# NVIDIA/audio-flamingo

Hardware: AMD Instinct MI355X
Metric: audio-sec/s + decoder tokens/s, AF3-7B bf16 train (higher is better)
Workload: dtype bf16; 1 GPU; AF3 (AF-Whisper 32L + Qwen2.5-7B 28L, MLP projector) bf16 train step fwd+bwd+AdamW, 30 s clips, S=1024; micro_batch_per_gpu=8, global_batch=8, seq_len=1024, parallelism=dp1, activation_checkpointing=False

## Files before the change

### audio-flamingo_amd/csrc/ceiling.hip

```cpp
#include "common.h"
#include "../../include/afk.h"

namespace {

constexpr int SEG = 16;

template <int MODE>
__global__ __launch_bounds__(512, 1) void mfma_ceiling_kernel(const bf16* __restrict__ src, float* __restrict__ sink, int iters) {
    extern __shared__ __attribute__((aligned(16))) char smem[];
    const int tid = threadIdx.x, lane = tid & 63, wave = tid >> 6;
    bf16x8 a[2][4], b[2][4];
    const bf16x8* s8 = (const bf16x8*)src;
#pragma unroll
    for (int i = 0; i < 2; ++i)
#pragma unroll
        for (int k = 0; k < 4; ++k) {
            a[i][k] = s8[((blockIdx.x * 8 + wave) * 16 + i * 4 + k) * 64 % 8192 + lane];
            b[i][k] = s8[((blockIdx.x * 8 + wave) * 16 + 8 + i * 4 + k) * 64 % 8192 + lane];
        }
    if (MODE == 1) {
        for (int i = tid; i < 4096; i += 512) ((bf16x8*)smem)[i] = s8[i];
        __syncthreads();
    }
    f32x16 acc[2][2];
#pragma unroll
    for (int i = 0; i < 2; ++i)
#pragma unroll
        for (int j = 0; j < 2; ++j)
#pragma unroll
            for (int e = 0; e < 16; ++e) acc[i][j][e] = 0.f;
    uint32_t lds = afk_lds_addr(smem) + lane * 16;
    for (int it = 0; it < iters; ++it) {
        if (MODE == 1) {
            const uint32_t base = lds + ((it * 12 * 1024) & 0xffff & ~0x3fff);
            afk_static_for<4>([&](auto K) {
                constexpr int k = decltype(K)::value;
                a[0][k] = afk_lds_b128<k * 1024>(base);
                a[1][k] = afk_lds_b128<(4 + k) * 1024>(base);
                b[k & 1][k] = afk_lds_b128<(8 + k) * 1024>(base);
            });
            afk_lds_wait0(a[0][0], a[0][1], a[0][2], a[0][3], a[1][0], a[1][1], a[1][2], a[1][3], b[0][0], b[1][1], b[0][2], b[1][3]);
        }
#pragma unroll
        for (int k = 0; k < 4; ++k)
#pragma unroll
            for (int i = 0; i < 2; ++i)
#pragma unroll
                for (int j = 0; j < 2; ++j) acc[i][j] = __builtin_amdgcn_mfma_f32_32x32x16_bf16(a[i][k], b[j][k], acc[i][j], 0, 0, 0);
    }
    float s = 0.f;
#pragma unroll
    for (int i = 0; i < 2; ++i)
#pragma unroll
        for (int j = 0; j < 2; ++j)
#pragma unroll
            for (int e = 0; e < 16; ++e) s += acc[i][j][e];
    if (s == 123.456f) sink[0] = s;
}

template <bool CHAIN>
__global__ __launch_bounds__(256, 1) void mfma_pacing_kernel(const bf16* __restrict__ src, float* __restrict__ sink, int iters) {
    const int lane = threadIdx.x & 63, wave = threadIdx.x >> 6;
    const bf16x8* s8 = (const bf16x8*)src;
    bf16x8 a[4], b[4];
#pragma unroll
    for (int k = 0; k < 4; ++k) {
        a[k] = s8[(wave * 8 + k) * 64 + lane];
        b[k] = s8[(wave * 8 + 4 + k) * 64 + lane];
    }
    f32x16 acc[4];
#pragma unroll
    for (int i = 0; i < 4; ++i)
#pragma unroll
        for (int e = 0; e < 16; ++e) acc[i][e] = 0.f;
    uint64_t t0, t1;
    asm volatile("s_waitcnt vmcnt(0)\n s_memtime %0\n s_waitcnt lgkmcnt(0)" : "=s"(t0)::"memory");
    for (int it = 0; it < iters; ++it) {
        if (CHAIN) {
#pragma unroll
            for (int i = 0; i < 4; ++i)
#pragma unroll
                for (int k = 0; k < 4; ++k) acc[i] = __builtin_amdgcn_mfma_f32_32x32x16_bf16(a[k], b[k], acc[i], 0, 0, 0);
        } else {
#pragma unroll
            for (int k = 0; k < 4; ++k)
#pragma unroll
                for (int i = 0; i < 4; ++i) acc[i] = __builtin_amdgcn_mfma_f32_32x32x16_bf16(a[k], b[k], acc[i], 0, 0, 0);
        }
    }
    float s = 0.f;
#pragma unroll
    for (int i = 0; i < 4; ++i)
#pragma unroll
        for (int e = 0; e < 16; ++e) s += acc[i][e];
    asm volatile("s_nop 0\n s_memtime %0\n s_waitcnt lgkmcnt(0)" : "=s"(t1) : "v"(s) : "memory");
    if (blockIdx.x == 0 && threadIdx.x == 0) sink[0] = (float)(t1 - t0) / (16.f * iters);
    if (s == 123.456f) sink[1] = s;
}

}

extern "C" int afk_mfma_ceiling(int mode, int nblocks, int iters, const void* operands, float* sink, double* host_flops, void* stream) {
    AFK_REQUIRE(mode >= 0 && mode <= 3, "afk_mfma_ceiling: mode %d (0 = register-resident operands, 1 = + LDS fragment reads, 2 / 3 = issue pacing of one wave per SIMD, "
                "independent / dependent accumulators: sink[0] = cycles per MFMA)", mode);
    AFK_REQUIRE(nblocks > 0 && iters > 0 && operands && sink, "afk_mfma_ceiling: bad arguments");
    hipStream_t s = (hipStream_t)stream;
    if (mode >= 2) {
        if (mode == 2) mfma_pacing_kernel<false><<<nblocks, 256, 0, s>>>((const bf16*)operands, sink, iters);
        else mfma_pacing_kernel<true><<<nblocks, 256, 0, s>>>((const bf16*)operands, sink, iters);
        AFK_LAUNCH_CHECK("afk_mfma_ceiling");
        if (host_flops) *host_flops = (double)nblocks * 4.0 * iters * 16 * 2.0 * 32 * 32 * 16;
        return AFK_OK;
    }
    if (mode == 0) {
        mfma_ceiling_kernel<0><<<nblocks, 512, 0, s>>>((const bf16*)operands, sink, iters);
    } else {
        static bool attr = false;
        if (!attr) {
            hipFuncSetAttribute((const void*)mfma_ceiling_kernel<1>, hipFuncAttributeMaxDynamicSharedMemorySize, 65536 + 16384);
            attr = true;
        }
        mfma_ceiling_kernel<1><<<nblocks, 512, 65536 + 16384, s>>>((const bf16*)operands, sink, iters);
    }
    AFK_LAUNCH_CHECK("afk_mfma_ceiling");
    if (host_flops) *host_flops = (double)nblocks * 8.0 * iters * SEG * 2.0 * 32 * 32 * 16;
    return AFK_OK;
}
```

### audio-flamingo_amd/csrc/gemm.hip

```cpp
#include "gemm_common.h"
#include <vector>
#include <mutex>

namespace {

constexpr int BM = 128, BN = 128, BK = 64;
constexpr int ROWB = BK * 2;
constexpr int STAGE_BYTES = (BM + BN) * ROWB;
constexpr int NSTAGE = 2;

__global__ __launch_bounds__(256, 2) void gemm_nt_bf16_k128(GemmArgs p) {
    extern __shared__ __attribute__((aligned(16))) char smem[];
    const int tid = threadIdx.x;
    const int lane = tid & 63;
    const int wave = __builtin_amdgcn_readfirstlane(tid >> 6);
    const int wm = wave >> 1, wn = wave & 1;
    const int hi = lane >> 5, l31 = lane & 31;

    int tm, tn;
    gemm_tile_of_block(p, tm, tn);
    const int m0 = tm * BM, n0 = tn * BN;

    const bf16* a_src[4];
    const bf16* b_src[4];
#pragma unroll
    for (int u = 0; u < 4; ++u) {
        const int unit = wave + 4 * u;
        const int rl = unit * 8 + (lane >> 3);
        const int chunk = (lane & 7) ^ ((rl >> 1) & 7);
        const int ra = min(m0 + rl, p.M - 1);
        const int rb = min(n0 + rl, p.N - 1);
        a_src[u] = p.A + (int64_t)ra * p.lda + chunk * 8;
        b_src[u] = p.B + (int64_t)rb * p.ldb + chunk * 8;
    }

    auto stage = [&](int buf, int kt) {
        char* sa = smem + buf * STAGE_BYTES;
        char* sb = sa + BM * ROWB;
        const int koff = kt * BK;
#pragma unroll
        for (int u = 0; u < 4; ++u) {
            const int unit = wave + 4 * u;
            __builtin_amdgcn_global_load_lds((gbl_void*)(a_src[u] + koff), (lds_void*)(sa + unit * 1024), 16, 0, 0);
        }
#pragma unroll
        for (int u = 0; u < 4; ++u) {
            const int unit = wave + 4 * u;
            __builtin_amdgcn_global_load_lds((gbl_void*)(b_src[u] + koff), (lds_void*)(sb + unit * 1024), 16, 0, 0);
        }
    };

    const int swz_l = (lane >> 1) & 7;
    int a_off[4], b_off[4];
#pragma unroll
    for (int s = 0; s < 4; ++s) {
        const int c = ((2 * s + hi) ^ swz_l) << 4;
        a_off[s] = (wm * 64 + l31) * ROWB + c;
        b_off[s] = (wn * 64 + l31) * ROWB + c;
    }

    f32x16 acc[2][2];
#pragma unroll
    for (int i = 0; i < 2; ++i)
#pragma unroll
        for (int j = 0; j < 2; ++j)
#pragma unroll
            for (int e = 0; e < 16; ++e) acc[i][j][e] = 0.f;

    int kt0 = 0, nkt = p.K / BK;
    if (p.splits > 1) {
        const int all = nkt, sp = blockIdx.y;
        kt0 = (int)((int64_t)all * sp / p.splits);
        nkt = (int)((int64_t)all * (sp + 1) / p.splits);
    }
    if (kt0 < nkt) stage(kt0 & 1, kt0);
    __syncthreads();
    for (int kt = kt0; kt < nkt; ++kt) {
        const int cur = kt & 1;
        if (kt + 1 < nkt) stage(cur ^ 1, kt + 1);
        const char* sa = smem + cur * STAGE_BYTES;
        const char* sb = sa + BM * ROWB;
#pragma unroll
        for (int s = 0; s < 4; ++s) {
            bf16x8 af[2], bfr[2];
#pragma unroll
            for (int i = 0; i < 2; ++i) af[i] = *(const bf16x8*)(sa + a_off[s] + i * 32 * ROWB);
#pragma unroll
            for (int j = 0; j < 2; ++j) bfr[j] = *(const bf16x8*)(sb + b_off[s] + j * 32 * ROWB);
#pragma unroll
            for (int i = 0; i < 2; ++i)
#pragma unroll
                for (int j = 0; j < 2; ++j)
                    acc[i][j] = __builtin_amdgcn_mfma_f32_32x32x16_bf16(bfr[j], af[i], acc[i][j], 0, 0, 0);
        }
        __syncthreads();
    }

#pragma unroll
    for (int i = 0; i < 2; ++i)
#pragma unroll
        for (int j = 0; j < 2; ++j) gemm_store_block32_body<-1>(p, m0 + wm * 64 + i * 32 + l31, n0 + wn * 64 + j * 32, hi, acc[i][j]);
}

#define AFK_GEMV_MAX_M 1
template <int MB, int R>
__global__ __launch_bounds__(256) void gemv_nt_bf16_kernel(GemmArgs p) {
    const int lane = threadIdx.x & 63, wave = threadIdx.x >> 6;
    const int n0 = (blockIdx.x * 4 + wave) * R;
    if (n0 >= p.N) return;
    const int kb_all = (p.K + 511) >> 9;
    const int kb0 = (int)((int64_t)kb_all * blockIdx.y / p.splits), kb1 = (int)((int64_t)kb_all * (blockIdx.y + 1) / p.splits);
    float acc[R][MB];
#pragma unroll
    for (int r = 0; r < R; ++r)
#pragma unroll
        for (int m = 0; m < MB; ++m) acc[r][m] = 0.f;
    const bf16* wrow[R];
#pragma unroll
    for (int r = 0; r < R; ++r) wrow[r] = p.B + (int64_t)min(n0 + r, p.N - 1) * p.ldb;
    for (int kb = kb0; kb < kb1; ++kb) {
        const int k = (kb << 9) + lane * 8;
        if (k < p.K) {
            bf16x8 wv[R], xv[MB];
#pragma unroll
            for (int r = 0; r < R; ++r) wv[r] = __builtin_nontemporal_load((const bf16x8*)(wrow[r] + k));
#pragma unroll
            for (int m = 0; m < MB; ++m) xv[m] = *(const bf16x8*)(p.A + (int64_t)min(m, p.M - 1) * p.lda + k);
#pragma unroll
            for (int r = 0; r < R; ++r)
#pragma unroll
                for (int m = 0; m < MB; ++m)
#pragma unroll
                    for (int e = 0; e < 4; ++e) {
                        const bf16x2 a = {wv[r][2 * e], wv[r][2 * e + 1]}, b = {xv[m][2 * e], xv[m][2 * e + 1]};
                        acc[r][m] = __builtin_amdgcn_fdot2_f32_bf16(a, b, acc[r][m], false);
                    }
        }
    }
    constexpr int V = R * MB;
    static_assert((V & (V - 1)) == 0 && V <= 64, "R*MB must be a power of two <= 64");
    float* v = &acc[0][0];
    int n = V;
#pragma unroll
    for (int sft = 5; sft >= 0; --sft) {
        const int st = 1 << sft;
        const bool up = (lane >> sft) & 1;
        if (n > 1) {
            const int h = n >> 1;
#pragma unroll
            for (int i = 0; i < V / 2; ++i)
                if (i < h) {
                    const float lo = v[i], hi_ = v[i + h];
                    v[i] = (up ? hi_ : lo) + __shfl_xor(up ? lo : hi_, st, 64);
                }
            n = h;
        } else {
            v[0] += __shfl_xor(v[0], st, 64);
        }
    }
    constexpr int LOGV = V == 64 ? 6 : V == 32 ? 5 : V == 16 ? 4 : V == 8 ? 3 : V == 4 ? 2 : V == 2 ? 1 : 0;
    const int idx = lane >> (6 - LOGV);
    const int r = idx / MB, m = idx % MB;
    if ((lane & ((64 >> LOGV) - 1)) == 0 && n0 + r < p.N && m < p.M) p.ws[((int64_t)blockIdx.y * p.M + m) * p.N + n0 + r] = v[0];
}

__global__ __launch_bounds__(256) void gemm_splitk_reduce_kernel(GemmArgs p) {
    const int n4 = p.N >> 2;
    const int64_t total = (int64_t)p.M * n4;
    for (int64_t t = (int64_t)blockIdx.x * blockDim.x + threadIdx.x; t < total; t += (int64_t)gridDim.x * blockDim.x) {
        const int m = (int)(t / n4), n = (int)(t % n4) * 4;
        const float* src = p.ws + (int64_t)m * p.N + n;
        f32x4 acc = *(const f32x4*)src;
        for (int sp = 1; sp < p.splits; ++sp) {
            const f32x4 x = *(const f32x4*)(src + (int64_t)sp * p.M * p.N);
#pragma unroll
            for (int e = 0; e < 4; ++e) acc[e] += x[e];
        }
        float v[4] = {acc[0], acc[1], acc[2], acc[3]};
        gemm_epilogue_store4(p, m, n, v);
    }
}

struct ProfState {
    std::mutex mu;
    bool on = false;
    std::vector<hipEvent_t> pool;
    size_t used = 0;
    double flops = 0.0;
    int64_t launches = 0;
    struct Rec { int M, N, K, variant; };
    std::vector<Rec> recs;
};
ProfState g_prof;
int g_variant = 0;
[[maybe_unused]] int g_256_impl = 2;
int g_gm = 0;
int g_wide = 1;

hipEvent_t prof_next_event() {
    if (g_prof.used == g_prof.pool.size()) {
        hipEvent_t e;
        hipEventCreate(&e);
        g_prof.pool.push_back(e);
    }
    return g_prof.pool[g_prof.used++];
}

}

extern "C" int afk_gemm_set_variant(int v) {
    const int gm = (v >> 8) & 255, base = v & 15;
#ifdef AFK_PROBES
    AFK_REQUIRE(base >= 0 && base <= 14, "afk_gemm_set_variant: 14 = persistent tile loop with the next tile's prologue issued ahead of the epilogue stores (round-4 probe), 13 = 256x256 ping-pong as a persistent tile loop, 0 auto, 1 = 128x128, 2 = 256x256 8-wave ping-pong, 3 = 256x256 4-wave (4, 5: its timing probes), 6 = 256x256 8-wave free-running BK=64 (7, 8, 9: probes), 10 = 8-wave free-running BK=32 ring-10 (11: probe)");
#else
    AFK_REQUIRE(base >= 0 && base <= 2, "afk_gemm_set_variant: variant %d is a probe / rejected schedule; this libafk.so was built without -DAFK_PROBES (make PROBES=1)", base);
    AFK_REQUIRE((gm & 0xc0) == 0, "afk_gemm_set_variant: gm bits 6 / 7 are timing probes (wrong results); this libafk.so was built without -DAFK_PROBES");
#endif
    g_gm = gm;
    g_wide = (v & 16) ? 0 : 1;
    g_variant = base;
    return AFK_OK;
}

extern "C" int afk_prof_enable(int on) {
    std::lock_guard<std::mutex> lk(g_prof.mu);
    g_prof.on = on != 0;
    return AFK_OK;
}

extern "C" int afk_prof_reset(void) {
    std::lock_guard<std::mutex> lk(g_prof.mu);
    g_prof.used = 0;
    g_prof.flops = 0.0;
    g_prof.launches = 0;
    g_prof.recs.clear();
    return AFK_OK;
}

extern "C" int afk_prof_collect(double* total_ms, double* total_flops, int64_t* launches) {
    std::lock_guard<std::mutex> lk(g_prof.mu);
    double ms = 0.0;
    for (size_t i = 0; i + 1 < g_prof.used; i += 2) {
        if (hipEventSynchronize(g_prof.pool[i + 1]) != hipSuccess)
            return afk_set_error(AFK_ERR_LAUNCH, "afk_prof_collect: event sync failed");
        float t = 0.f;
        if (hipEventElapsedTime(&t, g_prof.pool[i], g_prof.pool[i + 1]) != hipSuccess)
            return afk_set_error(AFK_ERR_LAUNCH, "afk_prof_collect: elapsed failed");
        ms += t;
    }
    if (total_ms) *total_ms = ms;
    if (total_flops) *total_flops = g_prof.flops;
    if (launches) *launches = g_prof.launches;
    return AFK_OK;
}

struct RopeEpi { const void *cos_t, *sin_t; const int* pos; int S, cols; const void *cos_lanes, *sin_lanes; };

static int gemm_impl(int trans_a, int trans_b, const void* A, int64_t lda, const void* B, int64_t ldb, void* C, int64_t ldc,
                     int M, int N, int K, const void* bias, const void* residual, int64_t ldr,
                     int res_mod, void* preact_out, float alpha, int flags, void* stream, int splits = 1, void* workspace = nullptr,
                     const RopeEpi* rope = nullptr) {
    AFK_REQUIRE(splits >= 1 && splits <= 64 && (splits == 1 || workspace), "afk_gemm_*_splitk: 1..64 splits, workspace required");
    AFK_REQUIRE(((flags & AFK_GEMM_ROPE) != 0) == (rope != nullptr), "afk_gemm: AFK_GEMM_ROPE belongs to afk_gemm_nt_bf16_rope");
    AFK_REQUIRE(splits == 1 || splits <= (K + BK - 1) / BK, "afk_gemm_*_splitk: more splits than K tiles");
    const bool gemv = workspace != nullptr && M <= AFK_GEMV_MAX_M && !trans_a && !trans_b;
    AFK_REQUIRE(!gemv || splits <= (K + 511) / 512, "afk_gemm_nt_bf16_splitk: M <= 16 streams K in blocks of 512: at most ceil(K/512) splits");
    AFK_REQUIRE(A && B && C, "afk_gemm_nt_bf16: null operand");
    AFK_REQUIRE(M > 0 && N > 0 && K > 0, "afk_gemm_nt_bf16: bad shape %d %d %d", M, N, K);
    AFK_REQUIRE(!trans_a || trans_b, "afk_gemm_bf16: A^T with k-contiguous B is not implemented (NT, NN, TN are)");
    AFK_REQUIRE(trans_a || K % BK == 0, "afk_gemm_nt_bf16: K=%d must be a multiple of %d (pad the operand)", K, BK);
    AFK_REQUIRE(!trans_b || (N % 8 == 0 && N >= 8), "afk_gemm_bf16: N=%d must be a multiple of 8 for a reduction-major B", N);
    AFK_REQUIRE(!trans_a || (M % 8 == 0 && M >= 8), "afk_gemm_bf16: M=%d must be a multiple of 8 for a reduction-major A", M);
    AFK_REQUIRE(N % 4 == 0, "afk_gemm_nt_bf16: N=%d must be a multiple of 4", N);
    AFK_REQUIRE(lda % 8 == 0 && ldb % 8 == 0 && ldc % 4 == 0, "afk_gemm_nt_bf16: leading dims must keep 16-B (A,B) / 8-B (C) alignment");
    AFK_REQUIRE(!(flags & AFK_GEMM_BIAS) || bias, "afk_gemm_nt_bf16: BIAS flag without bias");
    AFK_REQUIRE(!(flags & AFK_GEMM_RESIDUAL) || (residual && ldr % 4 == 0), "afk_gemm_nt_bf16: RESIDUAL flag without residual");
    AFK_REQUIRE(!(flags & AFK_GEMM_SWIGLU_FWD) || (flags == AFK_GEMM_SWIGLU_FWD && !trans_a && !trans_b && preact_out && N % 256 == 0 && splits == 1 &&
                                                     ldc % 8 == 0 && (uintptr_t)C % 16 == 0 && (uintptr_t)preact_out % 16 == 0),
                "afk_gemm_nt_bf16: SWIGLU_FWD needs the NT form, preact_out, N = 2I with I %% 128 == 0 and no other flag");
    AFK_REQUIRE(!(flags & AFK_GEMM_SWIGLU_BWD) || (residual && ldr % 4 == 0 && ldc >= 2 * (int64_t)N && flags == AFK_GEMM_SWIGLU_BWD && splits == 1),
                "afk_gemm: SWIGLU_BWD needs the gate|up tensor as `residual`, a [M, 2N] output and no other epilogue flag");
    AFK_REQUIRE(((uintptr_t)A % 16 == 0) && ((uintptr_t)B % 16 == 0) && ((uintptr_t)C % 8 == 0), "afk_gemm_nt_bf16: misaligned pointer");
    GemmArgs p;
    p.A = (const bf16*)A;
    p.B = (const bf16*)B;
    p.C = C;
    p.C2 = preact_out;
    p.bias = (const bf16*)bias;
    p.R = (const bf16*)residual;
    p.lda = lda;
    p.ldb = ldb;
    p.ldc = ldc;
    p.ldr = ldr;
    p.M = M;
    p.N = N;
    p.K = K;
    p.flags = flags;
    p.res_mod = res_mod;
    p.alpha = alpha;
    p.gm = g_gm;
    p.splits = splits;
    p.ws = (float*)workspace;
    p.rope_cos = rope ? (const bf16*)rope->cos_t : nullptr;
    p.rope_sin = rope ? (const bf16*)rope->sin_t : nullptr;
    p.rope_pos = rope ? rope->pos : nullptr;
    p.rope_S = rope ? rope->S : 1;
    p.rope_cols = rope ? rope->cols : 0;
    const bool lanes_ok = rope && rope->cos_lanes && rope->sin_lanes && !rope->pos && rope->S % 32 == 0;
    p.rope_cos_lanes = lanes_ok ? (const bf16*)rope->cos_lanes : nullptr;
    p.rope_sin_lanes = lanes_ok ? (const bf16*)rope->sin_lanes : nullptr;
    {
        const bool f32 = (flags & AFK_GEMM_OUT_F32) != 0;
        bool w = N % 8 == 0 && ldc % 8 == 0 && (uintptr_t)C % (f32 ? 32 : 16) == 0;
        if (flags & AFK_GEMM_BIAS) w = w && (uintptr_t)bias % 16 == 0;
        if (flags & (AFK_GEMM_RESIDUAL | AFK_GEMM_SWIGLU_BWD)) w = w && ldr % 8 == 0 && (uintptr_t)residual % 16 == 0;
        if (preact_out) w = w && (uintptr_t)preact_out % 16 == 0;
        p.wide = w && g_wide ? 1 : 0;
    }
    const int64_t tiles256 = afk_cdiv(M, 256) * afk_cdiv(N, 256);
    const bool use256 = !gemv && (trans_b || (flags & AFK_GEMM_SWIGLU_FWD) || (splits == 1 && (g_variant >= 2 || (g_variant == 0 && tiles256 >= 192))));
    if (rope && (!use256 || !p.wide || trans_a || trans_b || splits != 1))
        return afk_set_error(AFK_ERR_UNSUPPORTED, "afk_gemm_nt_bf16_rope: needs the 256 x 256 NT kernel (>= 192 tiles) in its 16-byte epilogue form; use "
                                                  "afk_gemm_nt_bf16 + afk_rope_inplace for this shape");
#ifdef AFK_PROBES
    static const int env_impl = [] {
        const char* e = getenv("AFK_GEMM256");
        return (e && e[0] == 'p' && e[1] == 'e') ? 13 : (e && e[0] == 'p') ? 2 : (e && e[0] == 'w') ? 3 : (e && e[0] == 'f') ? 10 : 0;
    }();
    const int impl256 = (flags & (AFK_GEMM_SWIGLU_FWD | AFK_GEMM_ROPE)) ? 2 : g_variant >= 2 ? g_variant : (env_impl ? env_impl : g_256_impl);
    const bool w4 = use256 && !trans_b && impl256 >= 3 && impl256 <= 9;
    const bool f8 = use256 && !trans_b && impl256 >= 10 && impl256 <= 12;
    const bool persist = use256 && !trans_b && impl256 == 13;
    const bool persist_q = use256 && !trans_b && impl256 == 14;
#endif
    if ((flags & AFK_GEMM_SWIGLU_FWD) && !p.wide)
        return afk_set_error(AFK_ERR_UNSUPPORTED, "afk_gemm_nt_bf16: SWIGLU_FWD needs the 16-byte epilogue form (aligned C / preact_out, ldc %% 8 == 0, "
                                                  "afk_gemm_set_variant bit 4 clear)");
    p.ntm = (int)afk_cdiv(M, use256 ? 256 : BM);
    p.ntn = (int)afk_cdiv(N, use256 ? 256 : BN);
    static bool attr_set = false;
    if (!attr_set) {
        hipFuncSetAttribute((const void*)gemm_nt_bf16_k128, hipFuncAttributeMaxDynamicSharedMemorySize, NSTAGE * STAGE_BYTES);
        attr_set = true;
    }
    hipStream_t st = (hipStream_t)stream;
    const int64_t nwg = (int64_t)p.ntm * p.ntn;
    AFK_REQUIRE(nwg < (1ll << 31), "afk_gemm_nt_bf16: grid too large");
    hipEvent_t e0 = nullptr, e1 = nullptr;
    bool prof = false;
    {
        std::lock_guard<std::mutex> lk(g_prof.mu);
        prof = g_prof.on;
        if (prof) {
            e0 = prof_next_event();
            e1 = prof_next_event();
            g_prof.flops += 2.0 * (double)M * (double)N * (double)K;
            g_prof.launches += 1;
            g_prof.recs.push_back({M, N, K, trans_b ? (trans_a ? 4 : 3) : (use256 ? 2 : 1)});
        }
    }
    afk_count(gemv ? AFK_CNT_GEMV : trans_b ? (trans_a ? AFK_CNT_GEMM_TN256 : AFK_CNT_GEMM_NN256) : use256 ? AFK_CNT_GEMM_NT256 : AFK_CNT_GEMM_NT128);
    if (splits > 1) afk_count(AFK_CNT_GEMM_SPLITK);
    if (prof) hipEventRecord(e0, st);
    if (gemv) {
        const dim3 grid((unsigned)afk_cdiv(N, 32), (unsigned)splits);
#define AFK_GEMV(MB_, R_) hipLaunchKernelGGL((gemv_nt_bf16_kernel<MB_, R_>), grid, dim3(256), 0, st, p)
        AFK_GEMV(1, 8);
#undef AFK_GEMV
        int g = (int)afk_cdiv((int64_t)M * (N / 4), 256);
        if (g > 2048) g = 2048;
        hipLaunchKernelGGL(gemm_splitk_reduce_kernel, dim3(g), dim3(256), 0, st, p);
    } else if (trans_b) {
        if (int e = afk_launch_gemm256t(p, trans_a, st)) return e;
        if (splits > 1) {
            int g = (int)afk_cdiv((int64_t)M * (N / 4), 256);
            if (g > 2048) g = 2048;
            hipLaunchKernelGGL(gemm_splitk_reduce_kernel, dim3(g), dim3(256), 0, st, p);
        }
    } else if (use256) {
#ifdef AFK_PROBES
        if (int e = persist_q ? afk_launch_gemm256q(p, st) : persist ? afk_launch_gemm256p(p, st) : f8 ? afk_launch_gemm256f8(p, impl256 - 10, st) : w4 ? afk_launch_gemm256w4(p, impl256 - 3, st) : afk_launch_gemm256(p, st)) return e;
#else
        if (int e = afk_launch_gemm256(p, st)) return e;
#endif
    } else {
        hipLaunchKernelGGL(gemm_nt_bf16_k128, dim3((unsigned)nwg, (unsigned)splits), dim3(256), NSTAGE * STAGE_BYTES, st, p);
        if (splits > 1) {
            int g = (int)afk_cdiv((int64_t)M * (N / 4), 256);
            if (g > 2048) g = 2048;
            hipLaunchKernelGGL(gemm_splitk_reduce_kernel, dim3(g), dim3(256), 0, st, p);
        }
    }
    if (prof) hipEventRecord(e1, st);
    AFK_LAUNCH_CHECK("afk_gemm_nt_bf16");
    return AFK_OK;
}

extern "C" int afk_gemm_nt_bf16(const void* A, int64_t lda, const void* B, int64_t ldb, void* C, int64_t ldc,
                                int M, int N, int K, const void* bias, const void* residual, int64_t ldr,
                                int res_mod, void* preact_out, float alpha, int flags, void* stream) {
    return gemm_impl(0, 0, A, lda, B, ldb, C, ldc, M, N, K, bias, residual, ldr, res_mod, preact_out, alpha, flags, stream);
}

extern "C" int afk_gemm_nt_bf16_rope(const void* A, int64_t lda, const void* B, int64_t ldb, void* C, int64_t ldc, int M, int N, int K, const void* bias,
                                     const void* cos_t, const void* sin_t, const int* pos, int S, int rope_cols, const void* cos_lanes, const void* sin_lanes,
                                     void* stream) {
    AFK_REQUIRE(cos_t && sin_t && (uintptr_t)cos_t % 16 == 0 && (uintptr_t)sin_t % 16 == 0, "afk_gemm_nt_bf16_rope: cos / sin tables (16-byte aligned) are required");
    AFK_REQUIRE(N % 256 == 0 && rope_cols >= 0 && rope_cols <= N && rope_cols % 256 == 0 && S > 0,
                "afk_gemm_nt_bf16_rope: N and rope_cols must be multiples of 256 (two 128-column heads per tile), S > 0");
    AFK_REQUIRE((cos_lanes == nullptr) == (sin_lanes == nullptr) && (!cos_lanes || ((uintptr_t)cos_lanes % 16 == 0 && (uintptr_t)sin_lanes % 16 == 0)),
                "afk_gemm_nt_bf16_rope: the lane-major tables come as a 16-byte aligned pair");
    const RopeEpi r = {cos_t, sin_t, pos, S, rope_cols, cos_lanes, sin_lanes};
    return gemm_impl(0, 0, A, lda, B, ldb, C, ldc, M, N, K, bias, nullptr, 0, 0, nullptr, 1.f, AFK_GEMM_ROPE | (bias ? AFK_GEMM_BIAS : 0), stream, 1, nullptr, &r);
}

extern "C" int afk_gemm_nt_bf16_splitk(const void* A, int64_t lda, const void* B, int64_t ldb, void* C, int64_t ldc, int M, int N, int K,
                                       const void* bias, const void* residual, int64_t ldr, int res_mod, void* preact_out, float alpha,
                                       int flags, int splits, void* workspace, void* stream) {
    return gemm_impl(0, 0, A, lda, B, ldb, C, ldc, M, N, K, bias, residual, ldr, res_mod, preact_out, alpha, flags, stream, splits, workspace);
}

extern "C" int afk_gemv_partials(const void* A, int64_t lda, const void* B, int64_t ldb, int M, int N, int K, int splits, float* workspace,
                                 void* stream) {
    AFK_REQUIRE(A && B && workspace && M >= 1 && M <= AFK_GEMV_MAX_M && N > 0 && K > 0 && K % 8 == 0 && lda % 8 == 0 && ldb % 8 == 0,
                "afk_gemv_partials: bad args (M <= %d, K %% 8 == 0)", AFK_GEMV_MAX_M);
    AFK_REQUIRE(splits >= 1 && splits <= (K + 511) / 512 && splits <= 64, "afk_gemv_partials: 1 <= splits <= ceil(K / 512)");
    GemmArgs p = {};
    p.A = (const bf16*)A; p.B = (const bf16*)B; p.lda = lda; p.ldb = ldb; p.M = M; p.N = N; p.K = K; p.splits = splits; p.ws = workspace;
    const dim3 grid((unsigned)afk_cdiv(N, 32), (unsigned)splits);
    hipStream_t st = (hipStream_t)stream;
    hipLaunchKernelGGL((gemv_nt_bf16_kernel<1, 8>), grid, dim3(256), 0, st, p);
    AFK_LAUNCH_CHECK("afk_gemv_partials");
    return AFK_OK;
}

extern "C" int afk_gemm_bf16_splitk(int trans_a, int trans_b, const void* A, int64_t lda, const void* B, int64_t ldb, void* C, int64_t ldc,
                                    int M, int N, int K, const void* bias, const void* residual, int64_t ldr, int res_mod, void* preact_out,
                                    float alpha, int flags, int splits, void* workspace, void* stream) {
    return gemm_impl(trans_a, trans_b, A, lda, B, ldb, C, ldc, M, N, K, bias, residual, ldr, res_mod, preact_out, alpha, flags, stream, splits,
                     workspace);
}

extern "C" int afk_gemm_bf16(int trans_a, int trans_b, const void* A, int64_t lda, const void* B, int64_t ldb, void* C,
                             int64_t ldc, int M, int N, int K, const void* bias, const void* residual, int64_t ldr,
                             int res_mod, void* preact_out, float alpha, int flags, void* stream) {
    return gemm_impl(trans_a, trans_b, A, lda, B, ldb, C, ldc, M, N, K, bias, residual, ldr, res_mod, preact_out, alpha, flags, stream);
}

extern "C" int afk_prof_dump(const char* host_path) {
    std::lock_guard<std::mutex> lk(g_prof.mu);
    FILE* f = fopen(host_path, "w");
    if (!f) return afk_set_error(AFK_ERR_ARG, "afk_prof_dump: cannot open %s", host_path);
    fprintf(f, "M,N,K,variant,ms\n");
    for (size_t i = 0; i < g_prof.recs.size() && 2 * i + 1 < g_prof.used; ++i) {
        float ms = 0.f;
        hipEventSynchronize(g_prof.pool[2 * i + 1]);
        hipEventElapsedTime(&ms, g_prof.pool[2 * i], g_prof.pool[2 * i + 1]);
        fprintf(f, "%d,%d,%d,%d,%.6f\n", g_prof.recs[i].M, g_prof.recs[i].N, g_prof.recs[i].K, g_prof.recs[i].variant, ms);
    }
    fclose(f);
    return AFK_OK;
}
```

### audio-flamingo_amd/csrc/gemm256.hip

```cpp
#include "gemm_common.h"

namespace {

constexpr int BM = 256, BN = 256, BK = 64;
constexpr int ROWB = 128;
constexpr int OP_BYTES = 256 * ROWB;
constexpr int BUF_BYTES = 2 * OP_BYTES;
constexpr int LDS_BYTES = 2 * BUF_BYTES;

#define AFK_VMCNT(n) asm volatile("s_waitcnt vmcnt(" #n ")" ::: "memory")
#define AFK_LGKMCNT0() asm volatile("s_waitcnt lgkmcnt(0)" ::: "memory")
#define AFK_BARRIER()                         \
    do {                                      \
        __builtin_amdgcn_sched_barrier(0);    \
        __builtin_amdgcn_s_barrier();         \
        __builtin_amdgcn_sched_barrier(0);    \
    } while (0)

template <int EPI>
__global__ __launch_bounds__(512, 1) void gemm_nt_bf16_k256(GemmArgs p) {
    extern __shared__ __attribute__((aligned(16))) char smem[];
    const int tid = threadIdx.x;
    const int lane = tid & 63;
    const int wave = __builtin_amdgcn_readfirstlane(tid >> 6);
    const int wm = wave >> 2, wn = wave & 3;
    const int hi = lane >> 5, l31 = lane & 31;

    int tm, tn;
    gemm_tile_of_block(p, tm, tn);
    const int m0 = tm * BM, n0 = tn * BN;

    const bf16* xsrc[6];
    int xdst[6];
    const bf16* ysrc[2];
    int ydst[2];
    {
        const int lrow = lane >> 3, pos = lane & 7;
#pragma unroll
        for (int j = 0; j < 6; ++j) {
            const int i = wave + 8 * j;
            const bool isB = i < 32;
            const int unit = isB ? i : ((i - 32) < 8 ? (i - 32) : (i - 32) + 8);
            const int rl = unit * 8 + lrow;
            const int chunk = pos ^ ((rl >> 1) & 7);
            if (isB) {
                const int r = (EPI == AFK_GEMM_SWIGLU_FWD) ? (rl < 128 ? tn * 128 + rl : (p.N >> 1) + tn * 128 + rl - 128) : min(n0 + rl, p.N - 1);
                xsrc[j] = p.B + (int64_t)r * p.ldb + chunk * 8;
            } else {
                const int r = min(m0 + rl, p.M - 1);
                xsrc[j] = p.A + (int64_t)r * p.lda + chunk * 8;
            }
            xdst[j] = (isB ? OP_BYTES : 0) + unit * 1024;
        }
#pragma unroll
        for (int j = 0; j < 2; ++j) {
            const int jj = wave + 8 * j;
            const int unit = jj < 8 ? 8 + jj : 16 + jj;
            const int rl = unit * 8 + lrow;
            const int chunk = pos ^ ((rl >> 1) & 7);
            const int r = min(m0 + rl, p.M - 1);
            ysrc[j] = p.A + (int64_t)r * p.lda + chunk * 8;
            ydst[j] = unit * 1024;
        }
    }
    auto issue_x = [&](int t) {
        char* base = smem + (t & 1) * BUF_BYTES;
        const int koff = t * BK;
#pragma unroll
        for (int j = 0; j < 6; ++j)
            __builtin_amdgcn_global_load_lds((gbl_void*)(xsrc[j] + koff), (lds_void*)(base + xdst[j]), 16, 0, 0);
    };
    auto issue_y = [&](int t) {
        char* base = smem + (t & 1) * BUF_BYTES;
        const int koff = t * BK;
#pragma unroll
        for (int j = 0; j < 2; ++j)
            __builtin_amdgcn_global_load_lds((gbl_void*)(ysrc[j] + koff), (lds_void*)(base + ydst[j]), 16, 0, 0);
    };

    const int swz_l = (lane >> 1) & 7;
    int koffb[4];
#pragma unroll
    for (int s = 0; s < 4; ++s) koffb[s] = ((2 * s + hi) ^ swz_l) << 4;
    const int a_row0 = (wm * 128 + l31) * ROWB;
    const int b_row0 = OP_BYTES + (wn * 64 + l31) * ROWB;

    f32x16 acc[4][2];
#pragma unroll
    for (int i = 0; i < 4; ++i)
#pragma unroll
        for (int j = 0; j < 2; ++j)
#pragma unroll
            for (int e = 0; e < 16; ++e) acc[i][j][e] = 0.f;

    const int T = p.K / BK;
    issue_x(0);
    issue_y(0);
    if (T > 1) {
        issue_x(1);
        AFK_VMCNT(8);
    } else {
        AFK_VMCNT(2);
    }
    AFK_BARRIER();
    if (wm == 1) AFK_BARRIER();

    bf16x8 bf[2][4], af[2][4];
#define AFK_MFMA4(ACC0, s)                                                                                         \
    do {                                                                                                           \
        _Pragma("unroll") for (int i_ = 0; i_ < 2; ++i_) _Pragma("unroll") for (int j_ = 0; j_ < 2; ++j_)          \
            acc[ACC0 + i_][j_] = __builtin_amdgcn_mfma_f32_32x32x16_bf16(bf[j_][s], af[i_][s], acc[ACC0 + i_][j_], 0, 0, 0); \
    } while (0)
    for (int t = 0; t < T; ++t) {
        const char* buf = smem + (t & 1) * BUF_BYTES;
        const int t1 = min(t + 1, T - 1), t2 = min(t + 2, T - 1);
        const int e1 = (t + 1) & 1, e2 = t & 1;
        const int64_t oy = (int64_t)t1 * BK, ox = (int64_t)t2 * BK;
        char* by = smem + e1 * BUF_BYTES;
        char* bx = smem + e2 * BUF_BYTES;
#pragma unroll
        for (int j = 0; j < 2; ++j)
#pragma unroll
            for (int s = 0; s < 4; ++s) bf[j][s] = *(const bf16x8*)(buf + b_row0 + j * 32 * ROWB + koffb[s]);
#pragma unroll
        for (int i = 0; i < 2; ++i)
#pragma unroll
            for (int s = 0; s < 4; ++s) af[i][s] = *(const bf16x8*)(buf + a_row0 + i * 32 * ROWB + koffb[s]);
        AFK_LGKMCNT0();
        AFK_VMCNT(6);
        AFK_BARRIER();
        __builtin_amdgcn_s_setprio(1);
        AFK_MFMA4(0, 0);
        __builtin_amdgcn_sched_barrier(0);
        __builtin_amdgcn_global_load_lds((gbl_void*)(ysrc[0] + oy), (lds_void*)(by + ydst[0]), 16, 0, 0);
        __builtin_amdgcn_sched_barrier(0);
        AFK_MFMA4(0, 1);
        __builtin_amdgcn_sched_barrier(0);
        __builtin_amdgcn_global_load_lds((gbl_void*)(ysrc[1] + oy), (lds_void*)(by + ydst[1]), 16, 0, 0);
        __builtin_amdgcn_sched_barrier(0);
        AFK_MFMA4(0, 2);
        AFK_MFMA4(0, 3);
        __builtin_amdgcn_s_setprio(0);
        AFK_VMCNT(8);
        AFK_BARRIER();
#pragma unroll
        for (int i = 0; i < 2; ++i)
#pragma unroll
            for (int s = 0; s < 4; ++s) af[i][s] = *(const bf16x8*)(buf + a_row0 + (i + 2) * 32 * ROWB + koffb[s]);
        AFK_LGKMCNT0();
        AFK_VMCNT(2);
        AFK_BARRIER();
        __builtin_amdgcn_s_setprio(1);
#pragma unroll
        for (int s = 0; s < 4; ++s) {
#pragma unroll
            for (int i = 0; i < 2; ++i) {
                acc[2 + i][0] = __builtin_amdgcn_mfma_f32_32x32x16_bf16(bf[0][s], af[i][s], acc[2 + i][0], 0, 0, 0);
                acc[2 + i][1] = __builtin_amdgcn_mfma_f32_32x32x16_bf16(bf[1][s], af[i][s], acc[2 + i][1], 0, 0, 0);
                const int piece = 2 * s + i;
                if (piece < 6) {
                    __builtin_amdgcn_sched_barrier(0);
                    __builtin_amdgcn_global_load_lds((gbl_void*)(xsrc[piece] + ox), (lds_void*)(bx + xdst[piece]), 16, 0, 0);
                    __builtin_amdgcn_sched_barrier(0);
                }
            }
        }
        __builtin_amdgcn_s_setprio(0);
        AFK_VMCNT(8);
        AFK_BARRIER();
    }
    AFK_VMCNT(0);
#undef AFK_MFMA4
    if (wm == 0) AFK_BARRIER();

    if constexpr (EPI == AFK_GEMM_SWIGLU_FWD) {
        typedef __attribute__((ext_vector_type(8))) __bf16 b8;
        const int I = p.N >> 1;
        const bool up = wn >= 2;
        const int feat0 = tn * 128 + (wn & 1) * 64;
        char* xch = smem + (wm * 2 + (wn & 1)) * 16384 + lane * 16;
        b8 pc[16];
#pragma unroll
        for (int i = 0; i < 4; ++i)
#pragma unroll
            for (int j = 0; j < 2; ++j)
#pragma unroll
                for (int t = 0; t < 2; ++t) {
                    b8 o;
#pragma unroll
                    for (int e = 0; e < 4; ++e) {
                        const auto r = __builtin_amdgcn_permlane32_swap(__float_as_uint(acc[i][j][8 * t + e]), __float_as_uint(acc[i][j][8 * t + 4 + e]), false, false);
                        o[e] = (bf16)(__uint_as_float(r[0]) * p.alpha);
                        o[4 + e] = (bf16)(__uint_as_float(r[1]) * p.alpha);
                    }
                    pc[(i * 2 + j) * 2 + t] = o;
                }
        if (up) {
#pragma unroll
            for (int q = 0; q < 16; ++q) *(b8*)(xch + q * 1024) = pc[q];
        }
        __syncthreads();
#pragma unroll
        for (int i = 0; i < 4; ++i) {
            const int m = m0 + wm * 128 + i * 32 + l31;
#pragma unroll
            for (int j = 0; j < 2; ++j)
#pragma unroll
                for (int t = 0; t < 2; ++t) {
                    const int q = (i * 2 + j) * 2 + t;
                    const int f = feat0 + j * 32 + 16 * t + 8 * hi;
                    if (!up) {
                        const b8 u = *(const b8*)(xch + q * 1024);
                        b8 h;
#pragma unroll
                        for (int e = 0; e < 8; ++e) {
                            const float gf = (float)pc[q][e];
                            h[e] = (bf16)(rbf(gf * sigmoid_f(gf)) * (float)u[e]);
                        }
                        if (m < p.M) *(b8*)((bf16*)p.C2 + (int64_t)m * I + f) = h;
                    }
                    if (m < p.M) *(b8*)((bf16*)p.C + (int64_t)m * p.ldc + (up ? I : 0) + f) = pc[q];
                }
        }
        return;
    }
    if constexpr (EPI >= 0 && (EPI & AFK_GEMM_ROPE) != 0) {
        typedef __attribute__((ext_vector_type(8))) __bf16 b8;
        const bool rot = n0 < p.rope_cols;
        char* mine = smem + (wm * 4 + wn) * 16384 + lane * 16;
        const char* theirs = smem + (wm * 4 + (wn ^ 1)) * 16384 + lane * 16;
        b8 pc[16];
#pragma unroll
        for (int i = 0; i < 4; ++i)
#pragma unroll
            for (int j = 0; j < 2; ++j)
#pragma unroll
                for (int t = 0; t < 2; ++t) {
                    const int n = n0 + wn * 64 + j * 32 + 16 * t + 8 * hi;
                    b8 bv;
                    if constexpr ((EPI & AFK_GEMM_BIAS) != 0) bv = *(const b8*)(p.bias + n);
                    b8 o;
#pragma unroll
                    for (int e = 0; e < 4; ++e) {
                        const auto r = __builtin_amdgcn_permlane32_swap(__float_as_uint(acc[i][j][8 * t + e]), __float_as_uint(acc[i][j][8 * t + 4 + e]), false, false);
                        float v0 = __uint_as_float(r[0]) * p.alpha, v1 = __uint_as_float(r[1]) * p.alpha;
                        if constexpr ((EPI & AFK_GEMM_BIAS) != 0) {
                            v0 += (float)bv[e];
                            v1 += (float)bv[4 + e];
                        }
                        o[e] = (bf16)v0;
                        o[4 + e] = (bf16)v1;
                    }
                    pc[(i * 2 + j) * 2 + t] = o;
                }
        if (rot) {
#pragma unroll
            for (int q = 0; q < 16; ++q) *(b8*)(mine + q * 1024) = pc[q];
        }
        __syncthreads();
#pragma unroll
        for (int i = 0; i < 4; ++i) {
            const int m = m0 + wm * 128 + i * 32 + l31;
            const int mc = min(m, p.M - 1);
            const int64_t pr = p.rope_pos ? p.rope_pos[mc] : mc % p.rope_S;
            const bool lanes = p.rope_cos_lanes != nullptr;
            const int64_t lbase = lanes ? (((int64_t)((m0 + wm * 128 + i * 32) % p.rope_S) >> 5) * 16 * 32 + l31) * 8 : 0;
#pragma unroll
            for (int j = 0; j < 2; ++j)
#pragma unroll
                for (int t = 0; t < 2; ++t) {
                    const int q = (i * 2 + j) * 2 + t;
                    const int cl = wn * 64 + j * 32 + 16 * t + 8 * hi;
                    b8 o = pc[q];
                    if (rot) {
                        const int d = cl & 127;
                        const b8 other = *(const b8*)(theirs + q * 1024);
                        const b8 c = lanes ? *(const b8*)(p.rope_cos_lanes + lbase + (d >> 3) * 256) : *(const b8*)(p.rope_cos + pr * 128 + d);
                        const b8 sn = lanes ? *(const b8*)(p.rope_sin_lanes + lbase + (d >> 3) * 256) : *(const b8*)(p.rope_sin + pr * 128 + d);
                        const float sg = (wn & 1) ? 1.f : -1.f;
#pragma unroll
                        for (int e = 0; e < 8; ++e)
                            o[e] = (bf16)(rbf_strict((float)pc[q][e] * (float)c[e]) + rbf_strict(sg * (float)other[e] * (float)sn[e]));
                    }
                    if (m < p.M) *(b8*)((bf16*)p.C + (int64_t)m * p.ldc + n0 + cl) = o;
                }
        }
        return;
    }
    if (AFK_GM_NOEPI(p)) return;
#pragma unroll
    for (int i = 0; i < 4; ++i)
#pragma unroll
        for (int j = 0; j < 2; ++j) gemm_store_block32<EPI>(p, m0 + wm * 128 + i * 32 + l31, n0 + wn * 64 + j * 32, hi, acc[i][j]);
}

}

#define AFK_EPI_LIST(X) X(0) X(AFK_GEMM_BIAS) X(AFK_GEMM_RESIDUAL) X(AFK_GEMM_BIAS | AFK_GEMM_RESIDUAL) X(AFK_GEMM_BIAS | AFK_GEMM_GELU) \
    X(AFK_GEMM_BIAS | AFK_GEMM_GELU | AFK_GEMM_RESIDUAL) X(AFK_GEMM_ACCUM) X(AFK_GEMM_SWIGLU_FWD) X(AFK_GEMM_SWIGLU_BWD) X(AFK_GEMM_ROPE) X(AFK_GEMM_ROPE | AFK_GEMM_BIAS) X(-1)

int afk_launch_gemm256(const GemmArgs& p, hipStream_t st) {
    static bool attr_set = false;
    if (!attr_set) {
#define AFK_SET(F)                                                                                                                       \
    if (hipFuncSetAttribute((const void*)gemm_nt_bf16_k256<(F)>, hipFuncAttributeMaxDynamicSharedMemorySize, LDS_BYTES) != hipSuccess) \
        return afk_set_error(AFK_ERR_LAUNCH, "gemm256: cannot reserve %d bytes of LDS", LDS_BYTES);
        AFK_EPI_LIST(AFK_SET)
#undef AFK_SET
        attr_set = true;
    }
    const int64_t nwg = (int64_t)p.ntm * p.ntn;
    const int f = (p.wide && p.splits <= 1) ? p.flags : -1;
    switch (f) {
#define AFK_CASE(F)                                                                                          \
    case (F):                                                                                                \
        if ((F) == -1) afk_count(AFK_CNT_GEMM_GENERIC);                                                      \
        hipLaunchKernelGGL(gemm_nt_bf16_k256<(F)>, dim3((unsigned)nwg), dim3(512), LDS_BYTES, st, p);        \
        break;
        AFK_EPI_LIST(AFK_CASE)
#undef AFK_CASE
        default:
            afk_count(AFK_CNT_GEMM_GENERIC);
            hipLaunchKernelGGL(gemm_nt_bf16_k256<-1>, dim3((unsigned)nwg), dim3(512), LDS_BYTES, st, p);
    }
    return AFK_OK;
}
```

### audio-flamingo_amd/csrc/gemm256t.hip

```cpp
#include "gemm_common.h"

namespace {

constexpr int BK = 64;
constexpr int OP_BYTES = 32768;
constexpr int BUF_BYTES = 2 * OP_BYTES;
constexpr int LDS_BYTES = 2 * BUF_BYTES;
constexpr int TROW = 512;

typedef __attribute__((address_space(3))) bf16x4 lds_bf16x4;

#define AFK_VMCNT(n) asm volatile("s_waitcnt vmcnt(" #n ")" ::: "memory")
#define AFK_LGKMCNT0() asm volatile("s_waitcnt lgkmcnt(0)" ::: "memory")
#define AFK_BARRIER()                         \
    do {                                      \
        __builtin_amdgcn_sched_barrier(0);    \
        __builtin_amdgcn_s_barrier();         \
        __builtin_amdgcn_sched_barrier(0);    \
    } while (0)
#define AFK_DMA_PTR(SRCPTR, DSTPTR)                                                                       \
    do {                                                                                                  \
        __builtin_amdgcn_sched_barrier(0);                                                                \
        __builtin_amdgcn_global_load_lds((gbl_void*)(SRCPTR), (lds_void*)(DSTPTR), 16, 0, 0);             \
        __builtin_amdgcn_sched_barrier(0);                                                                \
    } while (0)
#define MFMA(a, b, c) __builtin_amdgcn_mfma_f32_32x32x16_bf16(a, b, c, 0, 0, 0)

__device__ __forceinline__ int tswz(int r) { return ((r & 3) << 2) | ((r >> 2) & 3); }

__device__ __forceinline__ int tr_off(int tile32, int pc, int lane) {
    const int g = lane >> 4, i = lane & 15, hi = g >> 1;
    const int chunk = 4 * tile32 + 2 * (g & 1) + ((i & 3) >> 1);
    const int r = 8 * hi + (i >> 2) + 4 * pc;
    return r * TROW + ((chunk ^ tswz(r)) << 4) + 8 * (i & 1);
}
template <int S>
__device__ __forceinline__ bf16x8 tr_frag(uint32_t buf, int off0, int off1) {
    return afk_lds_tr_frag<S * 16 * TROW>(buf + off0, buf + off1);
}

struct TSrc {
    const bf16* base;
    int krow;
};
__device__ __forceinline__ TSrc tsrc(const bf16* mat, int unit, int col0, int ncols, int lane) {
    const int krow = 2 * unit + (lane >> 5);
    const int pos = lane & 31;
    const int chunk = pos ^ tswz(krow);
    const int col = min(col0 + chunk * 8, ncols - 8);
    TSrc s;
    s.base = mat + col;
    s.krow = krow;
    return s;
}

template <bool AT, int EPI>
__global__ __launch_bounds__(512, 1) void gemm_xt_bf16_k256(GemmArgs p) {
    extern __shared__ __attribute__((aligned(16))) char smem[];
    const int tid = threadIdx.x;
    const int lane = tid & 63;
    const int wave = __builtin_amdgcn_readfirstlane(tid >> 6);
    const int wm = wave >> 2, wn = wave & 3;
    const int hi = lane >> 5, l31 = lane & 31;

    int tm, tn;
    gemm_tile_of_block(p, tm, tn);
    const int m0 = tm * 256, n0 = tn * 256;
    int KL = p.K;
    const bf16* Abase = p.A;
    const bf16* Bbase = p.B;
    if (p.splits > 1) {
        const int tall = (p.K + BK - 1) / BK;
        const int t0 = (int)((int64_t)tall * blockIdx.y / p.splits), t1 = (int)((int64_t)tall * (blockIdx.y + 1) / p.splits);
        const int kbeg = t0 * BK;
        KL = min(p.K, t1 * BK) - kbeg;
        Abase += AT ? (int64_t)kbeg * p.lda : (int64_t)kbeg;
        Bbase += (int64_t)kbeg * p.ldb;
    }
    const int T = (KL + BK - 1) / BK;
    constexpr int NX = AT ? 4 : 6, NY = AT ? 4 : 2;

    const bf16* an_src[NX + NY];
    TSrc tr_src[NX + NY];
    int64_t tr_ld[NX + NY];
    int dst[NX + NY];
#pragma unroll
    for (int j = 0; j < NX + NY; ++j) {
        const bool isx = j < NX;
        const int jj = isx ? j : j - NX;
        an_src[j] = nullptr;
        tr_src[j].base = nullptr;
        tr_src[j].krow = 0;
        tr_ld[j] = 0;
        if (AT) {
            const bool isA = jj < 2;
            const int unit = (isx ? 0 : 16) + wave + 8 * (jj & 1);
            tr_src[j] = isA ? tsrc(Abase, unit, m0, p.M, lane) : tsrc(Bbase, unit, n0, p.N, lane);
            tr_ld[j] = isA ? p.lda : p.ldb;
            dst[j] = (isA ? 0 : OP_BYTES) + unit * 1024;
        } else if (isx && jj < 4) {
            const int unit = wave + 8 * jj;
            tr_src[j] = tsrc(Bbase, unit, n0, p.N, lane);
            tr_ld[j] = p.ldb;
            dst[j] = OP_BYTES + unit * 1024;
        } else {
            const int k = wave + 8 * (isx ? jj - 4 : jj);
            const int unit = isx ? (k < 8 ? k : k + 8) : (k < 8 ? 8 + k : 16 + k);
            const int rl = unit * 8 + (lane >> 3);
            const int chunk = (lane & 7) ^ ((rl >> 1) & 7);
            const int r = min(m0 + rl, p.M - 1);
            an_src[j] = Abase + (int64_t)r * p.lda + chunk * 8;
            dst[j] = unit * 1024;
        }
    }
    const bf16* tbase[NX + NY];
#pragma unroll
    for (int j = 0; j < NX + NY; ++j) tbase[j] = (AT || j < 4) ? tr_src[j].base + (int64_t)tr_src[j].krow * tr_ld[j] : nullptr;
    f32x16 acc[4][2];
#pragma unroll
    for (int i = 0; i < 4; ++i)
#pragma unroll
        for (int j = 0; j < 2; ++j)
#pragma unroll
            for (int e = 0; e < 16; ++e) acc[i][j][e] = 0.f;

    const bool ragged = (KL % BK) != 0;
  auto pipeline = [&](auto rag_) {
    constexpr bool RAG = decltype(rag_)::value;
    auto src_of = [&](int j, int t) -> const bf16* {
        const bool tr = AT || j < 4;
        if (tr) {
            if constexpr (RAG) {
                const int row = min(t * BK + tr_src[j].krow, KL - 1);
                return tr_src[j].base + (int64_t)row * tr_ld[j];
            } else {
                return tbase[j] + (int64_t)t * BK * tr_ld[j];
            }
        }
        return an_src[j] + (int64_t)t * BK;
    };
    auto issue = [&](int j, int t_src, int parity) { AFK_DMA_PTR(src_of(j, t_src), smem + parity * BUF_BYTES + dst[j]); };

    int tob[2][2], toa[4][2];
#pragma unroll
    for (int j = 0; j < 2; ++j)
#pragma unroll
        for (int pc = 0; pc < 2; ++pc) tob[j][pc] = OP_BYTES + tr_off(wn * 2 + j, pc, lane);
#pragma unroll
    for (int i = 0; i < 4; ++i)
#pragma unroll
        for (int pc = 0; pc < 2; ++pc) toa[i][pc] = AT ? tr_off(wm * 4 + i, pc, lane) : 0;
    const int swz_l = (lane >> 1) & 7;
    int koffb[4];
#pragma unroll
    for (int s = 0; s < 4; ++s) koffb[s] = ((2 * s + hi) ^ swz_l) << 4;
    const int a_row0 = (wm * 128 + l31) * 128;

#pragma unroll
    for (int j = 0; j < NX; ++j) issue(j, 0, 0);
#pragma unroll
    for (int j = 0; j < NY; ++j) issue(NX + j, 0, 0);
    {
        const int t1 = min(1, T - 1);
#pragma unroll
        for (int j = 0; j < NX; ++j) issue(j, t1, 1);
    }
    if (AT) AFK_VMCNT(8); else AFK_VMCNT(8);
    AFK_BARRIER();
    if (wm == 1) AFK_BARRIER();

    bf16x8 bf[2][4], af[AT ? 4 : 2][AT ? 2 : 4];
    const uint32_t lds0 = afk_lds_addr(smem);
    for (int t = 0; t < T; ++t) {
        const char* buf = smem + (t & 1) * BUF_BYTES;
        const uint32_t lbuf = lds0 + (t & 1) * BUF_BYTES;
        const int t1 = min(t + 1, T - 1), t2 = min(t + 2, T - 1);
        const int e1 = (t + 1) & 1, e2 = t & 1;
        if (!AT) {
#pragma unroll
            for (int j = 0; j < 2; ++j)
                afk_static_for<4>([&](auto s_) { constexpr int s = decltype(s_)::value; bf[j][s] = tr_frag<s>(lbuf, tob[j][0], tob[j][1]); });
#pragma unroll
            for (int i = 0; i < 2; ++i)
#pragma unroll
                for (int s = 0; s < 4; ++s) af[i][s] = *(const bf16x8*)(buf + a_row0 + i * 32 * 128 + koffb[s]);
            AFK_LGKMCNT0();
            AFK_VMCNT(6);
            AFK_BARRIER();
            __builtin_amdgcn_s_setprio(1);
#pragma unroll
            for (int s = 0; s < 4; ++s) {
#pragma unroll
                for (int i = 0; i < 2; ++i)
#pragma unroll
                    for (int j = 0; j < 2; ++j) acc[i][j] = MFMA(bf[j][s], af[i][s], acc[i][j]);
                if (s < 2) issue(NX + s, t1, e1);
            }
            __builtin_amdgcn_s_setprio(0);
            AFK_VMCNT(8);
            AFK_BARRIER();
#pragma unroll
            for (int i = 0; i < 2; ++i)
#pragma unroll
                for (int s = 0; s < 4; ++s) af[i][s] = *(const bf16x8*)(buf + a_row0 + (i + 2) * 32 * 128 + koffb[s]);
            AFK_LGKMCNT0();
            AFK_VMCNT(2);
            AFK_BARRIER();
            __builtin_amdgcn_s_setprio(1);
#pragma unroll
            for (int s = 0; s < 4; ++s) {
#pragma unroll
                for (int i = 0; i < 2; ++i) {
                    acc[2 + i][0] = MFMA(bf[0][s], af[i][s], acc[2 + i][0]);
                    acc[2 + i][1] = MFMA(bf[1][s], af[i][s], acc[2 + i][1]);
                    const int piece = 2 * s + i;
                    if (piece < 6) issue(piece, t2, e2);
                }
            }
            __builtin_amdgcn_s_setprio(0);
            AFK_VMCNT(8);
            AFK_BARRIER();
        } else {
            const int kvalid = KL - t * BK;
#pragma unroll
            for (int ph = 0; ph < 2; ++ph) {
                afk_static_for<2>([&](auto s_) {
                    constexpr int s = decltype(s_)::value;
                    if (ph == 0) {
#pragma unroll
                        for (int j = 0; j < 2; ++j) bf[j][s] = tr_frag<s>(lbuf, tob[j][0], tob[j][1]);
#pragma unroll
                        for (int i = 0; i < 4; ++i) af[i][s] = tr_frag<s>(lbuf, toa[i][0], toa[i][1]);
                    } else {
#pragma unroll
                        for (int j = 0; j < 2; ++j) bf[j][s] = tr_frag<2 + s>(lbuf, tob[j][0], tob[j][1]);
#pragma unroll
                        for (int i = 0; i < 4; ++i) af[i][s] = tr_frag<2 + s>(lbuf, toa[i][0], toa[i][1]);
                    }
                });
                AFK_LGKMCNT0();
                if (RAG && kvalid < BK) {
#pragma unroll
                    for (int s = 0; s < 2; ++s)
#pragma unroll
                        for (int e = 0; e < 8; ++e) {
                            const bool dead = 16 * (2 * ph + s) + 8 * hi + e >= kvalid;
#pragma unroll
                            for (int i = 0; i < 4; ++i)
                                if (dead) af[i][s][e] = (bf16)0.f;
                        }
                }
                AFK_VMCNT(4);
                AFK_BARRIER();
                __builtin_amdgcn_s_setprio(1);
#pragma unroll
                for (int s = 0; s < 2; ++s) {
#pragma unroll
                    for (int i = 0; i < 4; ++i) {
                        acc[i][0] = MFMA(bf[0][s], af[i][s], acc[i][0]);
                        acc[i][1] = MFMA(bf[1][s], af[i][s], acc[i][1]);
                        const int piece = 4 * s + i;
                        if ((piece & 1) == 0) {
                            if (ph == 0) issue(NX + (piece >> 1), t1, e1);
                            else issue(piece >> 1, t2, e2);
                        }
                    }
                }
                __builtin_amdgcn_s_setprio(0);
                AFK_VMCNT(8);
                AFK_BARRIER();
            }
        }
    }
    AFK_VMCNT(0);
    if (wm == 0) AFK_BARRIER();
  };
    if (ragged) pipeline(std::true_type{});
    else pipeline(std::false_type{});

#pragma unroll
    for (int i = 0; i < 4; ++i)
#pragma unroll
        for (int j = 0; j < 2; ++j) gemm_store_block32<EPI>(p, m0 + wm * 128 + i * 32 + l31, n0 + wn * 64 + j * 32, hi, acc[i][j]);
}

}

#define AFK_EPI_LIST(X) X(0) X(AFK_GEMM_ACCUM) X(-2) X(-1)

int afk_launch_gemm256t(const GemmArgs& p, int trans_a, hipStream_t st) {
    static bool attr_set = false;
    if (!attr_set) {
#define AFK_SET(F)                                                                                                                                \
    if (hipFuncSetAttribute((const void*)gemm_xt_bf16_k256<false, (F)>, hipFuncAttributeMaxDynamicSharedMemorySize, LDS_BYTES) != hipSuccess || \
        hipFuncSetAttribute((const void*)gemm_xt_bf16_k256<true, (F)>, hipFuncAttributeMaxDynamicSharedMemorySize, LDS_BYTES) != hipSuccess)    \
        return afk_set_error(AFK_ERR_LAUNCH, "gemm256t: cannot reserve %d bytes of LDS", LDS_BYTES);
        AFK_EPI_LIST(AFK_SET)
#undef AFK_SET
        attr_set = true;
    }
    const int64_t nwg = (int64_t)p.ntm * p.ntn;
    const unsigned ns = (unsigned)(p.splits > 1 ? p.splits : 1);
    const int f = p.splits > 1 ? -2 : (p.wide ? p.flags : -1);
    const dim3 grid((unsigned)nwg, ns);
    switch (f) {
#define AFK_CASE(F)                                                                                                   \
    case (F):                                                                                                         \
        if ((F) == -1) afk_count(AFK_CNT_GEMM_GENERIC);                                                               \
        if (trans_a) hipLaunchKernelGGL((gemm_xt_bf16_k256<true, (F)>), grid, dim3(512), LDS_BYTES, st, p);          \
        else hipLaunchKernelGGL((gemm_xt_bf16_k256<false, (F)>), grid, dim3(512), LDS_BYTES, st, p);                 \
        break;
        AFK_EPI_LIST(AFK_CASE)
#undef AFK_CASE
        default:
            afk_count(AFK_CNT_GEMM_GENERIC);
            if (trans_a) hipLaunchKernelGGL((gemm_xt_bf16_k256<true, -1>), grid, dim3(512), LDS_BYTES, st, p);
            else hipLaunchKernelGGL((gemm_xt_bf16_k256<false, -1>), grid, dim3(512), LDS_BYTES, st, p);
    }
    return AFK_OK;
}
```

### audio-flamingo_amd/csrc/gemm_common.h

```cpp
#pragma once
#include "common.h"
#include "../../include/afk.h"

struct GemmArgs {
    const bf16* A;
    const bf16* B;
    void* C;
    void* C2;
    const bf16* bias;
    const bf16* R;
    int64_t lda, ldb, ldc, ldr;
    int M, N, K;
    int ntm, ntn;
    int flags;
    int res_mod;
    float alpha;
    int gm;
    int splits;
    float* ws;
    int wide;
    const bf16* rope_cos;
    const bf16* rope_sin;
    const int* rope_pos;
    int rope_S, rope_cols;
    const bf16* rope_cos_lanes;
    const bf16* rope_sin_lanes;
};

#ifdef AFK_PROBES
#define AFK_GM_NOEPI(p) (((p).gm & 0x40) != 0)
#define AFK_GM_RAW(p) (((p).gm & 0x80) != 0)
#else
#define AFK_GM_NOEPI(p) false
#define AFK_GM_RAW(p) false
#endif

typedef __attribute__((address_space(3))) void lds_void;
typedef const __attribute__((address_space(1))) void gbl_void;

__device__ __forceinline__ void gemm_tile_of(const GemmArgs& p, int bid, int nwg, int& tm, int& tn) {
    const int xcd = bid & 7, idx = bid >> 3, q = nwg >> 3, r = nwg & 7;
    const int swz = AFK_GM_RAW(p) ? bid : (xcd < r ? xcd * (q + 1) : r * (q + 1) + (xcd - r) * q) + idx;
    const int GM = (p.gm & 0x3f) > 0 ? (p.gm & 0x3f) : 4;
    const int per_group = GM * p.ntn;
    const int g = swz / per_group, rem = swz - g * per_group;
    const int first_m = g * GM;
    const int gsz = min(p.ntm - first_m, GM);
    tm = first_m + rem % gsz;
    tn = rem / gsz;
}
__device__ __forceinline__ void gemm_tile_of_block(const GemmArgs& p, int& tm, int& tn) { gemm_tile_of(p, blockIdx.x, gridDim.x, tm, tn); }

template <int W, int F = -1>
__device__ __forceinline__ void gemm_epilogue_store(const GemmArgs& p, int m, int n, float* v) {
    typedef __attribute__((ext_vector_type(W))) __bf16 bvec;
    typedef __attribute__((ext_vector_type(W))) float fvec;
    const int flags = F >= 0 ? F : p.flags;
#pragma unroll
    for (int e = 0; e < W; ++e) v[e] *= p.alpha;
    if (flags & AFK_GEMM_BIAS) {
        const bvec bv = *(const bvec*)(p.bias + n);
#pragma unroll
        for (int e = 0; e < W; ++e) v[e] += (float)bv[e];
    }
    if (flags & AFK_GEMM_GELU) {
#pragma unroll
        for (int e = 0; e < W; ++e) v[e] = rbf(v[e]);
        if (p.C2) {
            bvec pre;
#pragma unroll
            for (int e = 0; e < W; ++e) pre[e] = (bf16)v[e];
            *(bvec*)((bf16*)p.C2 + (int64_t)m * p.ldc + n) = pre;
        }
#pragma unroll
        for (int e = 0; e < W; ++e) v[e] = gelu_f(v[e]);
    }
    if (flags & AFK_GEMM_SWIGLU_BWD) {
        const bvec gv = *(const bvec*)(p.R + (int64_t)m * p.ldr + n);
        const bvec uv = *(const bvec*)(p.R + (int64_t)m * p.ldr + p.N + n);
        bvec og, ou;
#pragma unroll
        for (int e = 0; e < W; ++e) {
            const float gf = (float)gv[e], uf = (float)uv[e], df = rbf(v[e]);
            const float s = sigmoid_f(gf);
            og[e] = (bf16)(df * uf * (s * (1.f + gf * (1.f - s))));
            ou[e] = (bf16)(df * (gf * s));
        }
        bf16* cp = (bf16*)p.C + (int64_t)m * p.ldc + n;
        *(bvec*)cp = og;
        *(bvec*)(cp + p.N) = ou;
        return;
    }
    if (flags & AFK_GEMM_RESIDUAL) {
        const int rm = p.res_mod > 0 ? m % p.res_mod : m;
        const bvec rv = *(const bvec*)(p.R + (int64_t)rm * p.ldr + n);
#pragma unroll
        for (int e = 0; e < W; ++e) v[e] = rbf(v[e]) + (float)rv[e];
    }
    if (flags & AFK_GEMM_OUT_F32) {
        float* cp = (float*)p.C + (int64_t)m * p.ldc + n;
        fvec o;
        if (flags & AFK_GEMM_ACCUM) {
            o = *(const fvec*)cp;
#pragma unroll
            for (int e = 0; e < W; ++e) o[e] += v[e];
        } else {
#pragma unroll
            for (int e = 0; e < W; ++e) o[e] = v[e];
        }
        *(fvec*)cp = o;
    } else {
        bf16* cp = (bf16*)p.C + (int64_t)m * p.ldc + n;
        if (flags & AFK_GEMM_ACCUM) {
            const bvec old = *(const bvec*)cp;
#pragma unroll
            for (int e = 0; e < W; ++e) v[e] += (float)old[e];
        }
        bvec o;
#pragma unroll
        for (int e = 0; e < W; ++e) o[e] = (bf16)v[e];
        *(bvec*)cp = o;
    }
}
__device__ __forceinline__ void gemm_epilogue_store4(const GemmArgs& p, int m, int n, float v[4]) { gemm_epilogue_store<4, -1>(p, m, n, v); }

template <int F>
__device__ __forceinline__ void gemm_store_block32_body(const GemmArgs& p, int m, int nb, int hi, const f32x16& acc);
static __device__ __noinline__ void gemm_store_block32_generic(const GemmArgs& p, int m, int nb, int hi, f32x16 acc) {
    gemm_store_block32_body<-1>(p, m, nb, hi, acc);
}
template <int F = -1>
__device__ __forceinline__ void gemm_store_block32(const GemmArgs& p, int m, int nb, int hi, const f32x16& acc) {
    if constexpr (F == -1) gemm_store_block32_generic(p, m, nb, hi, acc);
    else gemm_store_block32_body<F>(p, m, nb, hi, acc);
}
template <int F>
__device__ __forceinline__ void gemm_store_block32_body(const GemmArgs& p, int m, int nb, int hi, const f32x16& acc) {
    if (m >= p.M) return;
    if (F == -2 || (F == -1 && p.splits > 1)) {
#pragma unroll
        for (int q = 0; q < 4; ++q) {
            const int n = nb + 8 * q + 4 * hi;
            if (n >= p.N) continue;
            const f32x4 o = {acc[4 * q], acc[4 * q + 1], acc[4 * q + 2], acc[4 * q + 3]};
            *(f32x4*)(p.ws + ((int64_t)blockIdx.y * p.M + m) * p.N + n) = o;
        }
        return;
    }
    if constexpr (F == -2) return;
    if (F >= 0 || p.wide) {
#pragma unroll
        for (int t = 0; t < 2; ++t) {
            float v[8];
#pragma unroll
            for (int e = 0; e < 4; ++e) {
                const auto r = __builtin_amdgcn_permlane32_swap(__float_as_uint(acc[8 * t + e]), __float_as_uint(acc[8 * t + 4 + e]), false, false);
                v[e] = __uint_as_float(r[0]);
                v[4 + e] = __uint_as_float(r[1]);
            }
            const int n = nb + 16 * t + 8 * hi;
            if (n < p.N) gemm_epilogue_store<8, F>(p, m, n, v);
        }
        return;
    }
#pragma unroll
    for (int q = 0; q < 4; ++q) {
        const int n = nb + 8 * q + 4 * hi;
        if (n >= p.N) continue;
        float v[4] = {acc[4 * q], acc[4 * q + 1], acc[4 * q + 2], acc[4 * q + 3]};
        gemm_epilogue_store<4, F>(p, m, n, v);
    }
}

int afk_launch_gemm256(const GemmArgs& p, hipStream_t st);
int afk_launch_gemm256p(const GemmArgs& p, hipStream_t st);
int afk_launch_gemm256q(const GemmArgs& p, hipStream_t st);
int afk_launch_gemm256f8(const GemmArgs& p, int mode, hipStream_t st);
int afk_launch_gemm256w4(const GemmArgs& p, int mode, hipStream_t st);
int afk_launch_gemm256t(const GemmArgs& p, int trans_a, hipStream_t st);
```

### audio-flamingo_amd/ops.py

```python
from __future__ import annotations

import os

import torch

from . import _lib
from ._lib import AfkError

BF16 = torch.bfloat16

GEMM_BIAS, GEMM_GELU, GEMM_RESIDUAL, GEMM_OUT_F32, GEMM_ACCUM, GEMM_SWIGLU_BWD, GEMM_SWIGLU_FWD = 1, 2, 4, 8, 16, 32, 64


def _stream() -> int:
    return torch.cuda.current_stream().cuda_stream


def _p(t):
    return 0 if t is None else t.data_ptr()


def _chk(t: torch.Tensor, dtype=None, name="tensor"):
    if not t.is_cuda:
        raise AfkError(f"{name}: expected a HIP device tensor, got {t.device} (no CPU fallback in this package)")
    if dtype is not None and t.dtype != dtype:
        raise AfkError(f"{name}: expected dtype {dtype}, got {t.dtype}")
    return t


def pad64(n: int) -> int:
    return (n + 63) // 64 * 64


GEMM_FUSE_ROPE = os.environ.get("AFK_FUSE_ROPE_FWD", "1") != "0"


def gemm_nt_rope(a, b, bias, cos, sin, *, S, rope_cols, D, pos=None):
    M, N, K = a.shape[0], b.shape[0], a.shape[1]
    fused = (GEMM_FUSE_ROPE and D == 128 and N % 256 == 0 and rope_cols % 256 == 0 and K % 64 == 0 and ((M + 255) // 256) * (N // 256) >= 192
             and cos.data_ptr() % 16 == 0 and sin.data_ptr() % 16 == 0 and a.stride(1) == 1 and b.stride(1) == 1)
    if fused:
        _chk(a, BF16, "gemm a"), _chk(b, BF16, "gemm b"), _chk(cos, BF16, "rope cos"), _chk(sin, BF16, "rope sin")
        out = torch.empty((M, N), device=a.device, dtype=BF16)
        lanes = pos is None and S % 32 == 0 and cos.shape[0] >= S and sin.shape[0] >= S
        cl, sl = (_rope_lanes(cos, S, D, 1), _rope_lanes(sin, S, D, 1)) if lanes else (None, None)
        _lib.call("afk_gemm_nt_bf16_rope", a.data_ptr(), a.stride(0), b.data_ptr(), b.stride(0), out.data_ptr(), out.stride(0), M, N, K,
                  _p(bias), cos.data_ptr(), sin.data_ptr(), _p(pos), S, rope_cols, _p(cl), _p(sl), _stream())
        return out
    out = gemm_nt(a, b, bias=bias)
    rope_(out, cos, sin, S=S, nheads=rope_cols // D, D=D, pos=pos)
    return out


def gemm_nt(a, b, out=None, *, bias=None, residual=None, res_mod=0, gelu=False, preact_out=None, out_f32=False,
            accumulate=False, alpha=1.0, M=None, N=None, K=None, swiglu_bwd=None, swiglu_fwd_out=None):
    _chk(a, BF16, "gemm a"), _chk(b, BF16, "gemm b")
    assert a.dim() == 2 and b.dim() == 2 and a.stride(1) == 1 and b.stride(1) == 1
    M = a.shape[0] if M is None else M
    N = b.shape[0] if N is None else N
    K = a.shape[1] if K is None else K
    assert K <= a.shape[1] and K <= b.shape[1]
    if swiglu_fwd_out is not None:
        assert bias is None and residual is None and not gelu and not accumulate and not out_f32 and preact_out is None and swiglu_bwd is None
        _chk(swiglu_fwd_out, BF16, "gemm swiglu_fwd_out")
        assert N % 256 == 0 and swiglu_fwd_out.is_contiguous() and tuple(swiglu_fwd_out.shape) == (M, N // 2)
        if out is None:
            out = torch.empty((M, N), device=a.device, dtype=BF16)
        _lib.call("afk_gemm_nt_bf16", a.data_ptr(), a.stride(0), b.data_ptr(), b.stride(0), out.data_ptr(), out.stride(0), M, N, K, 0, 0, 0, 0,
                  swiglu_fwd_out.data_ptr(), float(alpha), GEMM_SWIGLU_FWD, _stream())
        return out
    if swiglu_bwd is not None:
        assert bias is None and residual is None and not gelu and not accumulate and not out_f32 and swiglu_bwd.shape[1] == 2 * N
        _chk(swiglu_bwd, BF16, "gemm swiglu_bwd")
        if out is None:
            out = torch.empty((M, 2 * N), device=a.device, dtype=BF16)
        _lib.call("afk_gemm_nt_bf16", a.data_ptr(), a.stride(0), b.data_ptr(), b.stride(0), out.data_ptr(), out.stride(0), M, N, K, 0,
                  swiglu_bwd.data_ptr(), swiglu_bwd.stride(0), 0, 0, float(alpha), GEMM_SWIGLU_BWD, _stream())
        return out
    if out is None:
        out = torch.empty((M, N), device=a.device, dtype=torch.float32 if out_f32 else BF16)
    assert out.dim() == 2 and out.stride(1) == 1 and out.shape[0] >= M and out.shape[1] >= N
    flags = 0
    if bias is not None:
        flags |= GEMM_BIAS
        _chk(bias, BF16, "gemm bias")
    if gelu:
        flags |= GEMM_GELU
    if residual is not None:
        flags |= GEMM_RESIDUAL
        _chk(residual, BF16, "gemm residual")
        assert residual.stride(-1) == 1
    if out.dtype == torch.float32:
        flags |= GEMM_OUT_F32
    if accumulate:
        flags |= GEMM_ACCUM
    if preact_out is not None:
        assert preact_out.stride(0) == out.stride(0) and preact_out.dtype == BF16
    splits = splitk_plan(M, N, K)
    if splits > 1 or M <= GEMV_MAX_M:
        ws = torch.empty(splits * M * N, device=a.device, dtype=torch.float32)
        _lib.call("afk_gemm_nt_bf16_splitk", a.data_ptr(), a.stride(0), b.data_ptr(), b.stride(0), out.data_ptr(), out.stride(0),
                  M, N, K, _p(bias), _p(residual), residual.stride(0) if residual is not None else 0, res_mod,
                  _p(preact_out), float(alpha), flags, splits, ws.data_ptr(), _stream())
        return out
    _lib.call("afk_gemm_nt_bf16", a.data_ptr(), a.stride(0), b.data_ptr(), b.stride(0), out.data_ptr(), out.stride(0),
              M, N, K, _p(bias), _p(residual), residual.stride(0) if residual is not None else 0, res_mod,
              _p(preact_out), float(alpha), flags, _stream())
    return out


GEMV_MAX_M = 1
if os.environ.get("AFK_GEMM_NARROW") == "1":
    _lib.call("afk_gemm_set_variant", 16)
SPLITK = os.environ.get("AFK_SPLITK", "1") != "0"


def splitk_plan(M, N, K):
    if M <= GEMV_MAX_M and SPLITK:
        blocks = (N + 31) // 32
        return max(1, min(16, (K + 511) // 512, (1536 + blocks - 1) // blocks))
    if not SPLITK or K < 1024:
        return 1
    t256 = ((M + 255) // 256) * ((N + 255) // 256)
    t128 = ((M + 127) // 128) * ((N + 127) // 128)
    if t256 >= 192 or t128 > 300:
        return 1
    return max(1, min(16, K // 256, (512 + t128 - 1) // t128))


def gemm(a, b, out=None, *, trans_a=False, trans_b=False, bias=None, residual=None, res_mod=0, gelu=False, preact_out=None,
         accumulate=False, alpha=1.0, _splits=None):
    _chk(a, BF16, "gemm a"), _chk(b, BF16, "gemm b")
    assert a.dim() == 2 and b.dim() == 2 and a.stride(1) == 1 and b.stride(1) == 1
    if trans_a:
        K, M = a.shape
    else:
        M, K = a.shape
    if trans_b:
        Kb, N = b.shape
    else:
        N, Kb = b.shape
    assert K == Kb, (a.shape, b.shape, trans_a, trans_b)
    if out is None:
        out = torch.empty((M, N), device=a.device, dtype=BF16)
    assert out.dim() == 2 and out.stride(1) == 1 and out.shape[0] >= M and out.shape[1] >= N
    flags = 0
    if bias is not None:
        flags |= GEMM_BIAS
    if gelu:
        flags |= GEMM_GELU
    if residual is not None:
        flags |= GEMM_RESIDUAL
    if out.dtype == torch.float32:
        flags |= GEMM_OUT_F32
    if accumulate:
        flags |= GEMM_ACCUM
    if _splits is None and trans_a and trans_b and PEEL_TAIL and bias is None and residual is None and not gelu and preact_out is None:
        plan = peel_plan_256(M, N, K)
        if plan is not None:
            axis, cut, s = plan
            kw = dict(trans_a=True, trans_b=True, accumulate=accumulate, alpha=alpha)
            if axis == 0:
                gemm(a[:, :cut], b, out[:cut], _splits=1, **kw)
                gemm(a[:, cut:M], b, out[cut:M], _splits=s, **kw)
            else:
                gemm(a, b[:, :cut], out[:, :cut], _splits=1, **kw)
                gemm(a, b[:, cut:N], out[:, cut:N], _splits=s, **kw)
            return out
    splits = _splits if _splits is not None else (splitk_plan_256(M, N, K) if trans_b else 1)
    if splits > 1:
        ws = torch.empty(splits * M * N, device=a.device, dtype=torch.float32)
        _lib.call("afk_gemm_bf16_splitk", int(trans_a), int(trans_b), a.data_ptr(), a.stride(0), b.data_ptr(), b.stride(0), out.data_ptr(),
                  out.stride(0), M, N, K, _p(bias), _p(residual), residual.stride(0) if residual is not None else 0, res_mod,
                  _p(preact_out), float(alpha), flags, splits, ws.data_ptr(), _stream())
        return out
    _lib.call("afk_gemm_bf16", int(trans_a), int(trans_b), a.data_ptr(), a.stride(0), b.data_ptr(), b.stride(0), out.data_ptr(),
              out.stride(0), M, N, K, _p(bias), _p(residual), residual.stride(0) if residual is not None else 0, res_mod,
              _p(preact_out), float(alpha), flags, _stream())
    return out


SPLITK_ROUND = int(os.environ.get("AFK_SPLITK_ROUND", "256"))
PEEL_TAIL = os.environ.get("AFK_PEEL_TAIL", "0") == "1"


def peel_plan_256(M, N, K):
    tm, tn = (M + 255) // 256, (N + 255) // 256
    T = tm * tn
    if T <= 256 or K < 2048:
        return None
    base = (T + 255) // 256
    best = None
    for axis, (t_long, t_other) in enumerate(((tm, tn), (tn, tm))):
        for r in range(1, 9):
            t_tail = r * t_other
            t_main = T - t_tail
            if r >= t_long or t_tail > 128:
                break
            sp = min(16, (K // 64) // 8, SPLITK_ROUND // t_tail)
            if sp < 2:
                continue
            cost = (t_main + 255) // 256 + 1.0 / sp + 0.08
            if cost < base - 0.3 and (best is None or cost < best[0]):
                best = (cost, axis, (t_long - r) * 256, sp)
    return None if best is None else best[1:]


def splitk_plan_256(M, N, K):
    if not SPLITK or K < 2048:
        return 1
    t256 = ((M + 255) // 256) * ((N + 255) // 256)
    if t256 >= 128:
        return 1
    return max(1, min(16, K // 512, SPLITK_ROUND // t256))


COLSUM_FUSED = os.environ.get("AFK_COLSUM_FUSED", "1") == "1"
_COLSUM_COUNTERS = {}


def _colsum_counters(dev, n):
    key = (dev.index, torch.cuda.current_stream(dev).cuda_stream)
    t = _COLSUM_COUNTERS.get(key)
    if t is None or t.numel() < n:
        t = _COLSUM_COUNTERS[key] = torch.zeros(max(n, 4096), device=dev, dtype=torch.int32)
    return t


def colsum(x, out, *, accumulate=False):
    rows, cols = x.shape
    ns = _lib.load().afk_colsum_slices(rows)
    ws = torch.empty(ns * cols, device=x.device, dtype=torch.float32)
    if COLSUM_FUSED:
        cnt = _colsum_counters(x.device, (cols + 63) // 64)
        _lib.call("afk_colsum_bf16_fused", x.data_ptr(), x.stride(0), rows, cols, out.data_ptr(), int(accumulate), ws.data_ptr(), cnt.data_ptr(), _stream())
    else:
        _lib.call("afk_colsum_bf16", x.data_ptr(), x.stride(0), rows, cols, out.data_ptr(), int(accumulate), ws.data_ptr(), _stream())
    return out


THIN_BLOCKS = 0


def transpose(x, out=None, *, rpad=None):
    _chk(x, BF16, "transpose x")
    assert x.dim() == 2 and x.stride(1) == 1
    R, C = x.shape
    rpad = pad64(R) if rpad is None else rpad
    if out is None:
        out = torch.empty((C, rpad), device=x.device, dtype=BF16)
    _lib.call("afk_transpose_bf16", x.data_ptr(), out.data_ptr(), R, C, rpad, x.stride(0), out.stride(0), 1, 1, 0, 0, 0, 0,
              THIN_BLOCKS, _stream())
    return out


def transpose_heads(x, B, S, H, D, ld, spad, out=None):
    _chk(x, BF16, "transpose_heads x")
    if out is None:
        out = torch.empty((B, H, D, spad), device=x.device, dtype=BF16)
    _lib.call("afk_transpose_bf16", x.data_ptr(), out.data_ptr(), S, D, spad, ld, spad, B, H, S * ld, D, H * D * spad,
              D * spad, 0, _stream())
    return out


def layernorm_fwd(x, w, b, eps=1e-5):
    _chk(x, BF16, "layernorm x")
    D = x.shape[-1]
    rows = x.numel() // D
    y = torch.empty_like(x)
    mean = torch.empty(rows, device=x.device, dtype=torch.float32)
    rstd = torch.empty(rows, device=x.device, dtype=torch.float32)
    _lib.call("afk_layernorm_fwd", x.data_ptr(), w.data_ptr(), b.data_ptr(), y.data_ptr(), mean.data_ptr(), rstd.data_ptr(),
              rows, D, float(eps), _stream())
    return y, mean, rstd


def _norm_ws(rows, D, device):
    nb = _lib.load().afk_norm_bwd_blocks(rows)
    return torch.empty(nb * 2 * D, device=device, dtype=torch.float32)


def layernorm_bwd(x, w, dy, mean, rstd, dw, db, *, dx_add=None, accumulate=False, colsum_out=None, colsum_accumulate=False):
    D = x.shape[-1]
    rows = x.numel() // D
    dx = torch.empty_like(x)
    if colsum_out is not None:
        assert dx_add is not None and D % 8 == 0 and D <= 4096
        nb = _lib.load().afk_norm_bwd_blocks(rows)
        ws = torch.empty(nb * 3 * D, device=x.device, dtype=torch.float32)
        _lib.call("afk_layernorm_bwd_colsum", x.data_ptr(), w.data_ptr(), dy.data_ptr(), mean.data_ptr(), rstd.data_ptr(), dx.data_ptr(), dx_add.data_ptr(),
                  dw.data_ptr(), db.data_ptr(), int(accumulate), colsum_out.data_ptr(), int(colsum_accumulate), ws.data_ptr(), rows, D, _stream())
        return dx
    ws = _norm_ws(rows, D, x.device)
    _lib.call("afk_layernorm_bwd", x.data_ptr(), w.data_ptr(), dy.data_ptr(), mean.data_ptr(), rstd.data_ptr(), dx.data_ptr(),
              _p(dx_add), dw.data_ptr(), db.data_ptr(), int(accumulate), ws.data_ptr(), rows, D, _stream())
    return dx


def rmsnorm_fwd(x, w, eps=1e-6):
    _chk(x, BF16, "rmsnorm x")
    D = x.shape[-1]
    rows = x.numel() // D
    y = torch.empty_like(x)
    rstd = torch.empty(rows, device=x.device, dtype=torch.float32)
    _lib.call("afk_rmsnorm_fwd", x.data_ptr(), w.data_ptr(), y.data_ptr(), rstd.data_ptr(), rows, D, float(eps), _stream())
    return y, rstd


def rmsnorm_bwd(x, w, dy, rstd, dw, *, dx_add=None, accumulate=False):
    D = x.shape[-1]
    rows = x.numel() // D
    dx = torch.empty_like(x)
    ws = _norm_ws(rows, D, x.device)
    _lib.call("afk_rmsnorm_bwd", x.data_ptr(), w.data_ptr(), dy.data_ptr(), rstd.data_ptr(), dx.data_ptr(), _p(dx_add),
              dw.data_ptr(), int(accumulate), ws.data_ptr(), rows, D, _stream())
    return dx


def gelu_fwd(x):
    y = torch.empty_like(_chk(x, BF16))
    _lib.call("afk_gelu_fwd", x.data_ptr(), y.data_ptr(), x.numel(), _stream())
    return y


def gelu_bwd(dy, pre, *, colsum_out=None, colsum_accumulate=False):
    dx = torch.empty_like(_chk(dy, BF16))
    if colsum_out is not None:
        rows, C = dy.shape
        ws = torch.empty(_lib.load().afk_gelu_bwd_colsum_parts(rows) * C, device=dy.device, dtype=torch.float32)
        _lib.call("afk_gelu_bwd_colsum", dy.data_ptr(), pre.data_ptr(), dx.data_ptr(), rows, C, colsum_out.data_ptr(), int(colsum_accumulate), ws.data_ptr(), _stream())
        return dx
    _lib.call("afk_gelu_bwd", dy.data_ptr(), pre.data_ptr(), dx.data_ptr(), dy.numel(), _stream())
    return dx


def silu_mul_fwd(gu):
    rows, I2 = _chk(gu, BF16).shape
    h = torch.empty((rows, I2 // 2), device=gu.device, dtype=BF16)
    _lib.call("afk_silu_mul_fwd", gu.data_ptr(), h.data_ptr(), rows, I2 // 2, _stream())
    return h


def silu_mul_bwd(gu, dh):
    rows, I2 = gu.shape
    dgu = torch.empty_like(gu)
    _lib.call("afk_silu_mul_bwd", gu.data_ptr(), dh.data_ptr(), dgu.data_ptr(), rows, I2 // 2, _stream())
    return dgu


def rope_(buf, cos, sin, *, S, nheads, D, pos=None, backward=False):
    _chk(buf, BF16, "rope buf")
    rows, ld = buf.shape[0], buf.stride(0)
    _lib.call("afk_rope_inplace", buf.data_ptr(), cos.data_ptr(), sin.data_ptr(), _p(pos), rows, S, ld, nheads, D,
              int(backward), _stream())
    return buf


def rotary_time(x, cos, sin, *, backward=False):
    _chk(x, BF16, "rotary_time x"), _chk(cos, torch.float32, "rotary_time cos"), _chk(sin, torch.float32, "rotary_time sin")
    rows, E = x.shape
    R = cos.shape[-1]
    assert x.is_contiguous() and cos.is_contiguous() and sin.is_contiguous() and cos.numel() == rows * R == sin.numel()
    y = torch.empty_like(x)
    _lib.call("afk_rotary_time", x.data_ptr(), cos.data_ptr(), sin.data_ptr(), y.data_ptr(), rows, E, R, int(backward), _stream())
    return y


def add(a, b, out=None):
    out = torch.empty_like(a) if out is None else out
    _lib.call("afk_add_bf16", a.data_ptr(), b.data_ptr(), out.data_ptr(), a.numel(), _stream())
    return out


def scale_add_(x, y, scale_dev, *, accumulate=False):
    _lib.call("afk_scale_add_bf16", x.data_ptr(), y.data_ptr(), x.numel(), _chk(scale_dev, torch.float32).data_ptr(),
              int(accumulate), _stream())
    return y


def cast_f32_bf16(x):
    out = torch.empty(x.shape, device=x.device, dtype=BF16)
    _lib.call("afk_cast_f32_bf16", _chk(x, torch.float32).data_ptr(), out.data_ptr(), x.numel(), _stream())
    return out


def rowsum(xt, C, out, *, accumulate=False):
    _lib.call("afk_rowsum_bf16", xt.data_ptr(), xt.stride(0), C, out.data_ptr(), xt.shape[0], int(accumulate), _stream())
    return out


def im2col_conv1(x):
    W, C, T = x.shape
    assert x.is_contiguous() and x.is_cuda
    col = torch.empty((W * T, 3 * C), device=x.device, dtype=BF16)
    _lib.call("afk_im2col_conv1", x.data_ptr(), int(x.dtype == torch.float32), col.data_ptr(), W, C, T, _stream())
    return col


def im2col_conv2(h, W, Tin, C):
    Tout = (Tin - 1) // 2 + 1
    col = torch.empty((W * Tout, 3 * C), device=h.device, dtype=BF16)
    _lib.call("afk_im2col_conv2", h.data_ptr(), col.data_ptr(), W, Tin, Tout, C, _stream())
    return col


def col2im_conv2(dcol, W, Tin, C):
    Tout = (Tin - 1) // 2 + 1
    dh = torch.empty((W * Tin, C), device=dcol.device, dtype=BF16)
    _lib.call("afk_col2im_conv2", dcol.data_ptr(), dh.data_ptr(), W, Tin, Tout, C, _stream())
    return dh


def conv_weight_to_gemm(w, out=None):
    Co, Ci, _ = w.shape
    out = torch.empty((Co, 3 * Ci), device=w.device, dtype=BF16) if out is None else out
    _lib.call("afk_conv_weight_permute", w.data_ptr(), out.data_ptr(), Co, Ci, 0, 0, _stream())
    return out


def conv_weight_grad_from_gemm(dwp, dw, *, accumulate=False):
    Co, Ci, _ = dw.shape
    _lib.call("afk_conv_weight_permute", dwp.data_ptr(), dw.data_ptr(), Co, Ci, 1, int(accumulate), _stream())
    return dw


def avgpool2_fwd(x, out_rows, C):
    y = torch.empty((out_rows, C), device=x.device, dtype=BF16)
    _lib.call("afk_avgpool2_fwd", x.data_ptr(), y.data_ptr(), out_rows, C, _stream())
    return y


def avgpool2_bwd(dy, out_rows, C):
    dx = torch.empty((out_rows * 2, C), device=dy.device, dtype=BF16)
    _lib.call("afk_avgpool2_bwd", dy.data_ptr(), dx.data_ptr(), out_rows, C, _stream())
    return dx


def placeholder_scan(ids, audio_id):
    ids = _chk(ids.contiguous(), torch.int64, "input_ids")
    n = ids.numel()
    src = torch.empty(n, device=ids.device, dtype=torch.int32)
    cnt = torch.empty(1, device=ids.device, dtype=torch.int32)
    _lib.call("afk_placeholder_scan", ids.data_ptr(), n, int(audio_id), src.data_ptr(), cnt.data_ptr(), _stream())
    return src, cnt


def embed_scatter_fwd(ids, src, embed, audio):
    n, H = ids.numel(), embed.shape[1]
    out = torch.empty((n, H), device=embed.device, dtype=BF16)
    _lib.call("afk_embed_scatter_fwd", ids.data_ptr(), _p(src), embed.data_ptr(), _p(audio), out.data_ptr(), n, H, _stream())
    return out


def embed_scatter_bwd(ids, src, dout, d_embed, d_audio, perm=None):
    n, H = ids.numel(), dout.shape[-1]
    if d_embed is not None and perm is None:
        perm = torch.sort(ids.reshape(-1), stable=True).indices.to(torch.int32)
    _lib.call("afk_embed_scatter_bwd", ids.data_ptr(), _p(src), dout.data_ptr(), _p(d_embed), _p(d_audio), _p(perm), n, H, _stream())


def _row_stat_buffer(B, H, S, spad, device, kernel_writes_tail=True):
    t = torch.empty((B, H, spad), device=device, dtype=torch.float32)
    if spad > S and not kernel_writes_tail:
        t[:, :, S:].zero_()
    return t


ATTN_PERSIST = os.environ.get("AFK_ATTN_PERSIST", "0") == "1"
_ATTN_QUEUES = {}


def _attn_queue(dev):
    key = (dev.index, torch.cuda.current_stream(dev).cuda_stream)
    t = _ATTN_QUEUES.get(key)
    if t is None:
        t = _ATTN_QUEUES[key] = torch.zeros(2, device=dev, dtype=torch.int32)
    return t


ATTN_FUSE_DELTA = os.environ.get("AFK_ATTN_FUSE_DELTA", "1") == "1"
ATTN_IMPL = "lds"


def _use_lds(D):
    return ATTN_IMPL == "lds" and D in (64, 128)


def attn_fwd(qkv, B, S, Hq, Hkv, D, *, scale, causal, kv_len=None, kv_lo=None):
    if kv_lo is not None and not (_use_lds(D) and causal):
        raise _lib.AfkError("attn_fwd: kv_lo (left padding) runs on the LDS-staged causal kernels only; use attn_interval_fwd")
    _chk(qkv, BF16, "qkv")
    ld = qkv.stride(0)
    spad = pad64(S)
    q = qkv
    k = qkv[:, Hq * D:]
    v = qkv[:, (Hq + Hkv) * D:]
    o = torch.empty((B * S, Hq * D), device=qkv.device, dtype=BF16)
    if _use_lds(D):
        lse = _row_stat_buffer(B, Hq, S, spad, qkv.device)
        if ATTN_PERSIST and kv_len is None and kv_lo is None and S % 128 == 0:
            _lib.call("afk_attn2_fwd_persistent", q.data_ptr(), S * ld, D, ld, k.data_ptr(), S * ld, D, ld, v.data_ptr(), S * ld, D, ld,
                      o.data_ptr(), S * Hq * D, D, Hq * D, lse.data_ptr(), None, None, B, Hq, Hkv, S, spad, D, float(scale),
                      int(causal), _attn_queue(qkv.device).data_ptr(), _stream())
            return o, lse
        _lib.call("afk_attn2_fwd", q.data_ptr(), S * ld, D, ld, k.data_ptr(), S * ld, D, ld, v.data_ptr(), S * ld, D, ld,
                  o.data_ptr(), S * Hq * D, D, Hq * D, lse.data_ptr(), _p(kv_len), _p(kv_lo), B, Hq, Hkv, S, spad, D, float(scale),
                  int(causal), _stream())
        return o, lse
    vt = transpose_heads(v, B, S, Hkv, D, ld, spad)
    lse = torch.empty((B, Hq, S), device=qkv.device, dtype=torch.float32)
    _lib.call("afk_attn_fwd", q.data_ptr(), S * ld, D, ld, k.data_ptr(), S * ld, D, ld, vt.data_ptr(), o.data_ptr(),
              S * Hq * D, D, Hq * D, lse.data_ptr(), _p(kv_len), B, Hq, Hkv, S, spad, D, float(scale), int(causal), _stream())
    return o, lse


ATTN_FUSE_ROPE_BWD = os.environ.get("AFK_FUSE_ROPE_BWD", "1") != "0"


_ROPE_LANES = {}


def _rope_lanes(table, S, D, form=0):
    import weakref

    key = (table.data_ptr(), table._version, int(table.shape[0]), D, form)
    hit = _ROPE_LANES.get(key)
    if hit is not None and hit[0]() is table:
        return hit[1]
    rows = int(table.shape[0])
    out = torch.empty(((rows + 31) // 32) * 32 * D, device=table.device, dtype=BF16)
    _lib.call("afk_rope_lanes_table", table.data_ptr(), out.data_ptr(), rows, D, form, _stream())
    if len(_ROPE_LANES) > 64:
        _ROPE_LANES.clear()
    _ROPE_LANES[key] = (weakref.ref(table), out)
    return out


def _attn_bwd_impl(qkv, o, do, lse, B, S, Hq, Hkv, D, *, scale, causal, kv_len=None, kv_lo=None, rope=None):
    if kv_lo is not None and not (_use_lds(D) and causal and lse.shape[-1] == pad64(S)):
        raise _lib.AfkError("attn_bwd: kv_lo (left padding) runs on the LDS-staged causal kernels only; use attn_interval_bwd")
    ld = qkv.stride(0)
    spad = pad64(S)
    q = qkv
    k = qkv[:, Hq * D:]
    v = qkv[:, (Hq + Hkv) * D:]
    dev = qkv.device
    ldo = Hq * D
    dqkv = torch.empty_like(qkv)
    ldd = dqkv.stride(0)
    dq = dqkv
    dk = dqkv[:, Hq * D:]
    dv = dqkv[:, (Hq + Hkv) * D:]
    if _use_lds(D) and lse.shape[-1] == spad:
        delta = _row_stat_buffer(B, Hq, S, spad, dev, kernel_writes_tail=ATTN_FUSE_DELTA)
        scratch = torch.empty((2, B * S, Hq * D), device=dev, dtype=BF16) if Hq != Hkv else None
        if ATTN_FUSE_DELTA and rope is not None and ATTN_FUSE_ROPE_BWD and rope[0].data_ptr() % 16 == 0 and rope[1].data_ptr() % 16 == 0:
            cos, sin, pos = rope
            _chk(cos, BF16, "rope cos"), _chk(sin, BF16, "rope sin")
            cl, sl = _rope_lanes(cos, S, D) if pos is None and cos.shape[0] >= S else None, _rope_lanes(sin, S, D) if pos is None and sin.shape[0] >= S else None
            _lib.call("afk_attn2_bwd_fused_rope", q.data_ptr(), S * ld, D, ld, k.data_ptr(), S * ld, D, ld, v.data_ptr(), S * ld, D, ld,
                      o.data_ptr(), S * ldo, D, ldo, do.data_ptr(), S * ldo, D, ldo, lse.data_ptr(), delta.data_ptr(), dq.data_ptr(), S * ldd, D, ldd,
                      dk.data_ptr(), S * ldd, D, ldd, dv.data_ptr(), S * ldd, D, ldd, _p(kv_len), _p(kv_lo), B, Hq, Hkv, S, spad, D,
                      float(scale), int(causal), _p(scratch), cos.data_ptr(), sin.data_ptr(), _p(pos), _p(cl), _p(sl), _stream())
            return dqkv, True
        if ATTN_FUSE_DELTA:
            _lib.call("afk_attn2_bwd_fused", q.data_ptr(), S * ld, D, ld, k.data_ptr(), S * ld, D, ld, v.data_ptr(), S * ld, D, ld,
                      o.data_ptr(), S * ldo, D, ldo, do.data_ptr(), S * ldo, D, ldo, lse.data_ptr(), delta.data_ptr(), dq.data_ptr(), S * ldd, D, ldd,
                      dk.data_ptr(), S * ldd, D, ldd, dv.data_ptr(), S * ldd, D, ldd, _p(kv_len), _p(kv_lo), B, Hq, Hkv, S, spad, D,
                      float(scale), int(causal), _p(scratch), _stream())
            return dqkv, False
        _lib.call("afk_attn2_delta", o.data_ptr(), S * ldo, D, ldo, do.data_ptr(), S * ldo, D, ldo, delta.data_ptr(), B, Hq, S,
                  spad, D, _stream())
        _lib.call("afk_attn2_bwd", q.data_ptr(), S * ld, D, ld, k.data_ptr(), S * ld, D, ld, v.data_ptr(), S * ld, D, ld,
                  do.data_ptr(), S * ldo, D, ldo, lse.data_ptr(), delta.data_ptr(), dq.data_ptr(), S * ldd, D, ldd,
                  dk.data_ptr(), S * ldd, D, ldd, dv.data_ptr(), S * ldd, D, ldd, _p(kv_len), _p(kv_lo), B, Hq, Hkv, S, spad, D,
                  float(scale), int(causal), _p(scratch), _stream())
        return dqkv, False
    delta = torch.empty((B, Hq, S), device=dev, dtype=torch.float32)
    _lib.call("afk_attn_delta", o.data_ptr(), S * ldo, D, ldo, do.data_ptr(), S * ldo, D, ldo, delta.data_ptr(), B, Hq, S, D,
              _stream())
    qt = transpose_heads(q, B, S, Hq, D, ld, spad)
    kt = transpose_heads(k, B, S, Hkv, D, ld, spad)
    dot = transpose_heads(do, B, S, Hq, D, ldo, spad)
    _lib.call("afk_attn_bwd", q.data_ptr(), S * ld, D, ld, k.data_ptr(), S * ld, D, ld, v.data_ptr(), S * ld, D, ld,
              do.data_ptr(), S * ldo, D, ldo, qt.data_ptr(), kt.data_ptr(), dot.data_ptr(), lse.data_ptr(), delta.data_ptr(),
              dq.data_ptr(), S * ldd, D, ldd, dk.data_ptr(), S * ldd, D, ldd, dv.data_ptr(), S * ldd, D, ldd, _p(kv_len),
              B, Hq, Hkv, S, spad, D, float(scale), int(causal), _stream())
    return dqkv, False


def attn_bwd(qkv, o, do, lse, B, S, Hq, Hkv, D, *, scale, causal, kv_len=None, kv_lo=None, rope=None):
    dqkv, rotated = _attn_bwd_impl(qkv, o, do, lse, B, S, Hq, Hkv, D, scale=scale, causal=causal, kv_len=kv_len, kv_lo=kv_lo, rope=rope)
    if rope is not None and not rotated:
        rope_(dqkv, rope[0], rope[1], S=S, nheads=Hq + Hkv, D=D, pos=rope[2], backward=True)
    return dqkv


def xattn_fwd(q, k, v, krange, B, Sq, Sk, Hq, Hkv, D, scale):
    sqp, skp = pad64(Sq), pad64(Sk)
    vt = transpose_heads(v, B, Sk, Hkv, D, v.stride(0), skp)
    o = torch.empty((B * Sq, Hq * D), device=q.device, dtype=BF16)
    lse = torch.empty((B, Hq, Sq), device=q.device, dtype=torch.float32)
    _lib.call("afk_xattn_fwd", q.data_ptr(), Sq * q.stride(0), D, q.stride(0), k.data_ptr(), Sk * k.stride(0), D, k.stride(0),
              vt.data_ptr(), o.data_ptr(), Sq * Hq * D, D, Hq * D, lse.data_ptr(), 0, _p(krange), B, Hq, Hkv, Sq, Sk, sqp, skp, D,
              float(scale), _stream())
    return o, lse


def xattn_bwd(q, k, v, o, do, lse, krange, B, Sq, Sk, Hq, Hkv, D, scale, dq, dk, dv):
    dev = q.device
    sqp, skp = pad64(Sq), pad64(Sk)
    ldo = Hq * D
    delta = torch.empty((B, Hq, Sq), device=dev, dtype=torch.float32)
    _lib.call("afk_attn_delta", o.data_ptr(), Sq * ldo, D, ldo, do.data_ptr(), Sq * ldo, D, ldo, delta.data_ptr(), B, Hq, Sq, D, _stream())
    qt = transpose_heads(q, B, Sq, Hq, D, q.stride(0), sqp)
    kt = transpose_heads(k, B, Sk, Hkv, D, k.stride(0), skp)
    dot = transpose_heads(do, B, Sq, Hq, D, ldo, sqp)
    _lib.call("afk_xattn_bwd", q.data_ptr(), Sq * q.stride(0), D, q.stride(0), k.data_ptr(), Sk * k.stride(0), D, k.stride(0),
              v.data_ptr(), Sk * v.stride(0), D, v.stride(0), do.data_ptr(), Sq * ldo, D, ldo, qt.data_ptr(), kt.data_ptr(),
              dot.data_ptr(), lse.data_ptr(), delta.data_ptr(), dq.data_ptr(), Sq * dq.stride(0), D, dq.stride(0),
              dk.data_ptr(), Sk * dk.stride(0), D, dk.stride(0), dv.data_ptr(), Sk * dv.stride(0), D, dv.stride(0), 0, _p(krange),
              B, Hq, Hkv, Sq, Sk, sqp, skp, D, float(scale), _stream())


def attn_interval_fwd(qkv, krange, B, S, Hq, Hkv, D, *, scale):
    _chk(qkv, BF16, "qkv")
    return xattn_fwd(qkv, qkv[:, Hq * D:], qkv[:, (Hq + Hkv) * D:], krange, B, S, S, Hq, Hkv, D, scale)


def attn_interval_bwd(qkv, o, do, lse, krange, B, S, Hq, Hkv, D, *, scale):
    dqkv = torch.empty_like(qkv)
    xattn_bwd(qkv, qkv[:, Hq * D:], qkv[:, (Hq + Hkv) * D:], o, do, lse, krange, B, S, S, Hq, Hkv, D, scale,
              dqkv, dqkv[:, Hq * D:], dqkv[:, (Hq + Hkv) * D:])
    return dqkv


def gather_rows(x, rows):
    _chk(x, BF16, "gather_rows x")
    assert x.is_contiguous() and rows.dtype == torch.int64
    return embed_scatter_fwd(rows, None, x, None)


def scatter_rows(src, rows, M):
    out = torch.zeros((M, src.shape[1]), device=src.device, dtype=BF16)
    perm = torch.arange(rows.numel(), device=src.device, dtype=torch.int32)
    embed_scatter_bwd(rows, None, src, out, None, perm=perm)
    return out


def decode_sample(logits, *, temperature=1.0, top_k=0, top_p=1.0, seed=0, u=None, step_base=None, step_off=0, out=None, probs_out=None, kept_out=None,
                  tokens_out=None, tok_off=0, state=None, emb=None, x_out=None):
    _chk(logits, torch.float32, "decode_sample logits")
    if logits.dim() != 2 or logits.stride(1) != 1:
        raise AfkError(f"decode_sample logits: [B, V] with unit column stride, got {tuple(logits.shape)} strides {logits.stride()}")
    B, V = logits.shape
    if out is None:
        out = torch.empty(B, device=logits.device, dtype=torch.int64)
    for t_, dt, n, name in ((out, torch.int64, B, "out"), (u, torch.float32, B, "u"), (kept_out, torch.int32, B, "kept_out"), (step_base, torch.int32, 1, "step_base"),
                            (tokens_out, torch.int64, 1, "tokens_out"), (state, torch.int32, 4, "state")):
        if t_ is not None:
            _chk(t_, dt, f"decode_sample {name}")
            if t_.numel() < n or not t_.is_contiguous():
                raise AfkError(f"decode_sample {name}: a contiguous tensor of at least {n} elements, got {tuple(t_.shape)}")
    if probs_out is not None:
        _chk(probs_out, torch.float32, "decode_sample probs_out")
        if probs_out.shape != logits.shape or probs_out.stride(1) != 1:
            raise AfkError(f"decode_sample probs_out: {tuple(logits.shape)} with unit column stride, got {tuple(probs_out.shape)}")
    H = 0
    if state is not None:
        if emb is None or x_out is None:
            raise AfkError("decode_sample: state needs emb and x_out (the embedding row of the token is the next step's input)")
        _chk(emb, BF16, "decode_sample emb"), _chk(x_out, BF16, "decode_sample x_out")
        H = emb.shape[1]
        if x_out.numel() < H or not x_out.is_contiguous() or V > emb.shape[0]:
            raise AfkError(f"decode_sample: x_out holds {x_out.numel()} elements, emb is {tuple(emb.shape)} for V = {V}")
    seed = int(seed) & (2 ** 64 - 1)
    _lib.call("afk_decode_sample", logits.data_ptr(), logits.stride(0), B, V, float(temperature), int(top_k or 0), float(top_p), _p(u),
              seed - 2 ** 64 if seed >= 2 ** 63 else seed, _p(step_base), int(step_off), out.data_ptr(), _p(probs_out),
              probs_out.stride(0) if probs_out is not None else 0, _p(kept_out), _p(tokens_out), int(tok_off), _p(state), _p(emb),
              emb.stride(0) if emb is not None else 0, H, _p(x_out), _stream())
    return out


def count_valid(labels):
    out = torch.empty(1, device=labels.device, dtype=torch.float32)
    _lib.call("afk_count_valid", labels.data_ptr(), labels.numel(), out.data_ptr(), _stream())
    return out


def ce_fwd_bwd_(logits, shift_labels, row_loss, denom, *, upstream=1.0, write_grad=True):
    rows, V = logits.shape
    _lib.call("afk_ce_fwd_bwd", logits.data_ptr(), logits.stride(0), rows, V, shift_labels.data_ptr(), row_loss.data_ptr(),
              denom.data_ptr(), float(upstream), int(write_grad), _stream())


def loss_reduce(row_loss, denom, loss, *, accumulate=False):
    _lib.call("afk_loss_reduce", row_loss.data_ptr(), row_loss.numel(), denom.data_ptr(), loss.data_ptr(), int(accumulate),
              _stream())
    return loss


def adamw_step(master, m, v, grad, param, *, lr, beta1, beta2, eps, weight_decay, step, grad_scale=1.0, max_blocks=0, gate=None, hyper=None):
    _lib.call("afk_adamw_step", master.data_ptr(), m.data_ptr(), v.data_ptr(), grad.data_ptr(), param.data_ptr(), param.numel(),
              float(lr), float(beta1), float(beta2), float(eps), float(weight_decay), int(step), float(grad_scale),
              int(max_blocks), _p(gate), _p(hyper), _stream())


def adamw_step_t(master, m, v, grad, param, shadow, N, K, *, lr, beta1, beta2, eps, weight_decay, step, grad_scale=1.0, max_blocks=0, gate=None, hyper=None):
    _lib.call("afk_adamw_step_t", master.data_ptr(), m.data_ptr(), v.data_ptr(), grad.data_ptr(), param.data_ptr(), shadow.data_ptr(), int(N), int(K),
              shadow.stride(0), float(lr), float(beta1), float(beta2), float(eps), float(weight_decay), int(step), float(grad_scale), int(max_blocks),
              _p(gate), _p(hyper), _stream())


def adamw16_step(m, v, grad, param, *, lr, beta1, beta2, eps, weight_decay, step, grad_scale=1.0, max_blocks=0, gate=None, hyper=None):
    for t, what in ((m, "adamw16 m"), (v, "adamw16 v"), (grad, "adamw16 grad"), (param, "adamw16 param")):
        _chk(t, BF16, what)
        if t.numel() != param.numel():
            raise AfkError(f"{what}: {t.numel()} elements, param has {param.numel()}")
    _lib.call("afk_adamw16_step", m.data_ptr(), v.data_ptr(), grad.data_ptr(), param.data_ptr(), param.numel(),
              float(lr), float(beta1), float(beta2), float(eps), float(weight_decay), int(step), float(grad_scale),
              int(max_blocks), _p(gate), _p(hyper), _stream())


def adamw16_step_t(m, v, grad, param, shadow, N, K, *, lr, beta1, beta2, eps, weight_decay, step, grad_scale=1.0, max_blocks=0, gate=None, hyper=None):
    for t, what in ((m, "adamw16_t m"), (v, "adamw16_t v"), (grad, "adamw16_t grad"), (param, "adamw16_t param")):
        _chk(t, BF16, what)
        if t.numel() != int(N) * int(K):
            raise AfkError(f"{what}: {t.numel()} elements, [N, K] = [{N}, {K}]")
    _chk(shadow, BF16, "adamw16_t shadow")
    if shadow.shape[0] < int(K) or shadow.stride(0) < int(N):
        raise AfkError(f"adamw16_t shadow: {tuple(shadow.shape)} (row stride {shadow.stride(0)}) cannot hold [K, N] = [{K}, {N}]")
    _lib.call("afk_adamw16_step_t", m.data_ptr(), v.data_ptr(), grad.data_ptr(), param.data_ptr(), shadow.data_ptr(), int(N), int(K),
              shadow.stride(0), float(lr), float(beta1), float(beta2), float(eps), float(weight_decay), int(step), float(grad_scale), int(max_blocks),
              _p(gate), _p(hyper), _stream())


def sumsq_workspace_floats() -> int:
    return int(_lib.load().afk_sumsq_workspace_floats())


def sumsq_(x, acc, *, gate=None, ws=None):
    _chk(x, BF16, "sumsq x")
    if ws is None:
        ws = torch.empty(_lib.load().afk_sumsq_workspace_floats(), device=x.device, dtype=torch.float32)
    _lib.call("afk_sumsq_bf16", x.data_ptr(), x.numel(), _chk(acc, torch.float32).data_ptr(), _p(gate), ws.data_ptr(), _stream())
    return acc


def clip_coef_(sumsq, coef, *, max_norm, scale=1.0, norm_out=None):
    _lib.call("afk_clip_coef", _chk(sumsq, torch.float32).data_ptr(), sumsq.numel(), float(scale), float(max_norm), coef.data_ptr(), _p(norm_out), _stream())


def set_f32(dst, values):
    v = [float(x) for x in values] + [0.0] * (4 - len(values))
    _lib.call("afk_set_f32", _chk(dst, torch.float32).data_ptr(), len(values), v[0], v[1], v[2], v[3], _stream())


def gemm_set_variant(v: int):
    _lib.call("afk_gemm_set_variant", int(v))


KERNEL_FAMILIES = ("gemm_nt128", "gemm_nt256", "gemm_nn256", "gemm_tn256", "gemm_splitk", "gemv", "attn2_fwd_d64", "attn2_fwd_d128",
                   "attn2_bwd_d64", "attn2_bwd_d128", "gqa_reduce", "xattn_fwd", "xattn_bwd", "attn1_fwd", "attn1_bwd", "gemm_generic_epilogue")


def kernel_counts(reset: bool = False) -> dict:
    import ctypes

    buf = (ctypes.c_int64 * len(KERNEL_FAMILIES))()
    _lib.call("afk_kernel_counts", ctypes.addressof(buf), len(KERNEL_FAMILIES))
    if reset:
        _lib.call("afk_kernel_counts_reset")
    return dict(zip(KERNEL_FAMILIES, list(buf)))


def prof_enable(on: bool):
    _lib.call("afk_prof_enable", int(on))


def prof_reset():
    _lib.call("afk_prof_reset")


def prof_collect():
    import ctypes
    ms, fl, n = ctypes.c_double(), ctypes.c_double(), ctypes.c_int64()
    _lib.call("afk_prof_collect", ctypes.addressof(ms), ctypes.addressof(fl), ctypes.addressof(n))
    return ms.value, fl.value, n.value
```

### include/afk.h

```cpp
#ifndef AFK_H
#define AFK_H
#include <stdint.h>
#ifdef __cplusplus
extern "C" {
#endif

int afk_version(void);
const char* afk_last_error(void);
const char* afk_build_id(void);
int afk_has_probes(void);

#define AFK_CNT_GEMM_NT128 0
#define AFK_CNT_GEMM_NT256 1
#define AFK_CNT_GEMM_NN256 2
#define AFK_CNT_GEMM_TN256 3
#define AFK_CNT_GEMM_SPLITK 4
#define AFK_CNT_GEMV 5
#define AFK_CNT_ATTN2_FWD_D64 6
#define AFK_CNT_ATTN2_FWD_D128 7
#define AFK_CNT_ATTN2_BWD_D64 8
#define AFK_CNT_ATTN2_BWD_D128 9
#define AFK_CNT_GQA_REDUCE 10
#define AFK_CNT_XATTN_FWD 11
#define AFK_CNT_XATTN_BWD 12
#define AFK_CNT_ATTN1_FWD 13
#define AFK_CNT_ATTN1_BWD 14
#define AFK_CNT_GEMM_GENERIC 15
#define AFK_CNT_MAX 16
int afk_kernel_counts(int64_t* host_out, int n);
int afk_kernel_counts_reset(void);

int afk_prof_enable(int on);
int afk_prof_reset(void);
int afk_prof_collect(double* host_total_ms, double* host_total_flops, int64_t* host_launches);
int afk_prof_dump(const char* host_path);

int afk_gemm_set_variant(int variant);
#define AFK_GEMM_BIAS 1
#define AFK_GEMM_GELU 2
#define AFK_GEMM_RESIDUAL 4
#define AFK_GEMM_OUT_F32 8
#define AFK_GEMM_ACCUM 16
#define AFK_GEMM_SWIGLU_BWD 32
#define AFK_GEMM_ROPE 128
#define AFK_GEMM_SWIGLU_FWD 64
int afk_gemm_nt_bf16(const void* A, int64_t lda, const void* B, int64_t ldb, void* C, int64_t ldc,
                     int M, int N, int K, const void* bias, const void* residual, int64_t ldr,
                     int res_mod, void* preact_out, float alpha, int flags, void* stream);
int afk_gemm_bf16(int trans_a, int trans_b, const void* A, int64_t lda, const void* B, int64_t ldb, void* C,
                  int64_t ldc, int M, int N, int K, const void* bias, const void* residual, int64_t ldr,
                  int res_mod, void* preact_out, float alpha, int flags, void* stream);
int afk_gemm_nt_bf16_rope(const void* A, int64_t lda, const void* B, int64_t ldb, void* C, int64_t ldc, int M, int N, int K, const void* bias,
                          const void* cos_t, const void* sin_t, const int* pos, int S, int rope_cols, const void* cos_lanes, const void* sin_lanes, void* stream);
int afk_gemm_nt_bf16_splitk(const void* A, int64_t lda, const void* B, int64_t ldb, void* C, int64_t ldc, int M, int N, int K,
                            const void* bias, const void* residual, int64_t ldr, int res_mod, void* preact_out, float alpha,
                            int flags, int splits, void* workspace, void* stream);
int afk_gemm_bf16_splitk(int trans_a, int trans_b, const void* A, int64_t lda, const void* B, int64_t ldb, void* C, int64_t ldc,
                         int M, int N, int K, const void* bias, const void* residual, int64_t ldr, int res_mod, void* preact_out,
                         float alpha, int flags, int splits, void* workspace, void* stream);


int afk_norm_bwd_blocks(int64_t rows);
int afk_layernorm_fwd(const void* x, const void* w, const void* b, void* y, float* mean, float* rstd,
                      int64_t rows, int D, float eps, void* stream);
int afk_layernorm_bwd(const void* x, const void* w, const void* dy, const float* mean, const float* rstd,
                      void* dx, const void* dx_add, void* dw, void* db, int accumulate, float* workspace,
                      int64_t rows, int D, void* stream);
int afk_rmsnorm_fwd(const void* x, const void* w, void* y, float* rstd, int64_t rows, int D, float eps, void* stream);
int afk_gelu_bwd_colsum_parts(int64_t rows);
int afk_gelu_bwd_colsum(const void* dy, const void* pre, void* dx, int64_t rows, int C, void* colsum, int colsum_accumulate, float* workspace, void* stream);
int afk_layernorm_bwd_colsum(const void* x, const void* w, const void* dy, const float* mean, const float* rstd, void* dx, const void* dx_add, void* dw, void* db,
                             int accumulate, void* colsum, int colsum_accumulate, float* workspace, int64_t rows, int D, void* stream);
int afk_rmsnorm_bwd(const void* x, const void* w, const void* dy, const float* rstd, void* dx, const void* dx_add,
                    void* dw, int accumulate, float* workspace, int64_t rows, int D, void* stream);

int afk_transpose_bf16(const void* in, void* out, int R, int C, int Rpad, int64_t ld_in, int64_t ld_out, int nb1,
                       int nb2, int64_t bs1_in, int64_t bs2_in, int64_t bs1_out, int64_t bs2_out, int max_blocks, void* stream);
int afk_gelu_fwd(const void* x, void* y, int64_t n, void* stream);
int afk_gelu_bwd(const void* dy, const void* pre, void* dx, int64_t n, void* stream);
int afk_silu_mul_fwd(const void* gu, void* h, int64_t rows, int I, void* stream);
int afk_silu_mul_bwd(const void* gu, const void* dh, void* dgu, int64_t rows, int I, void* stream);
int afk_rope_inplace(void* buf, const void* cos_t, const void* sin_t, const int* pos, int64_t rows, int S, int ld,
                     int nheads, int D, int backward, void* stream);
int afk_add_bf16(const void* a, const void* b, void* out, int64_t n, void* stream);
int afk_cast_f32_bf16(const float* in, void* out, int64_t n, void* stream);
int afk_scale_add_bf16(const void* x, void* y, int64_t n, const float* scale_dev, int accumulate, void* stream);
int afk_rowsum_bf16(const void* in, int64_t ld, int C, void* out, int rows, int accumulate, void* stream);

int afk_colsum_slices(int64_t rows);
int afk_colsum_bf16(const void* in, int64_t ld, int64_t rows, int cols, void* out, int accumulate, float* workspace, void* stream);
int afk_colsum_bf16_fused(const void* in, int64_t ld, int64_t rows, int cols, void* out, int accumulate, float* workspace, int* counters, void* stream);

int afk_relu_fwd(const void* x, void* y, int64_t n, void* stream);
int afk_relu_bwd(const void* dy, const void* y, void* dx, int64_t n, void* stream);
int afk_gate_fwd(const void* x, const void* h, const void* alpha, int alpha_is_vector, const int* gate, void* y, int64_t rows,
                 int D, void* stream);
int afk_gate_bwd(const void* dy, const void* h, const void* alpha, int alpha_is_vector, const int* gate, void* dh,
                 float* fws, void* dalpha, int accumulate, int64_t rows, int D, void* stream);

int afk_im2col_conv1(const void* x, int x_is_f32, void* col, int W, int C, int T, void* stream);
int afk_im2col_conv2(const void* h, void* col, int W, int Tin, int Tout, int C, void* stream);
int afk_col2im_conv2(const void* dcol, void* dh, int W, int Tin, int Tout, int C, void* stream);
int afk_conv_weight_permute(const void* in, void* out, int Co, int Ci, int dir, int accumulate, void* stream);
int afk_avgpool2_fwd(const void* x, void* y, int64_t out_rows, int C, void* stream);
int afk_avgpool2_bwd(const void* dy, void* dx, int64_t out_rows, int C, void* stream);

int afk_placeholder_scan(const int64_t* ids, int64_t n, int64_t audio_id, int* src, int* n_audio, void* stream);
int afk_embed_scatter_fwd(const int64_t* ids, const int* src, const void* embed, const void* audio, void* out,
                          int64_t n, int H, void* stream);
int afk_embed_scatter_bwd(const int64_t* ids, const int* src, const void* dout, void* d_embed, void* d_audio,
                          const int* perm, int64_t n, int H, void* stream);

int afk_attn_fwd(const void* Q, int64_t q_bs, int64_t q_hs, int64_t q_rs, const void* K, int64_t k_bs, int64_t k_hs,
                 int64_t k_rs, const void* Vt, void* O, int64_t o_bs, int64_t o_hs, int64_t o_rs, float* LSE,
                 const int* kv_len, int B, int Hq, int Hkv, int S, int Spad, int D, float scale, int causal, void* stream);
int afk_attn_delta(const void* O, int64_t o_bs, int64_t o_hs, int64_t o_rs, const void* dO, int64_t do_bs,
                   int64_t do_hs, int64_t do_rs, float* delta, int B, int H, int S, int D, void* stream);
int afk_attn_bwd(const void* Q, int64_t q_bs, int64_t q_hs, int64_t q_rs, const void* K, int64_t k_bs, int64_t k_hs,
                 int64_t k_rs, const void* V, int64_t v_bs, int64_t v_hs, int64_t v_rs, const void* dO,
                 int64_t do_bs, int64_t do_hs, int64_t do_rs, const void* Qt, const void* Kt, const void* dOt,
                 const float* LSE, const float* delta, void* dQ, int64_t dq_bs, int64_t dq_hs, int64_t dq_rs,
                 void* dK, int64_t dk_bs, int64_t dk_hs, int64_t dk_rs, void* dV, int64_t dv_bs, int64_t dv_hs,
                 int64_t dv_rs, const int* kv_len, int B, int Hq, int Hkv, int S, int Spad, int D, float scale,
                 int causal, void* stream);

int afk_xattn_fwd(const void* Q, int64_t q_bs, int64_t q_hs, int64_t q_rs, const void* K, int64_t k_bs, int64_t k_hs,
                  int64_t k_rs, const void* Vt, void* O, int64_t o_bs, int64_t o_hs, int64_t o_rs, float* LSE,
                  const int* kv_len, const int* krange, int B, int Hq, int Hkv, int Sq, int Sk, int Sqpad, int Skpad,
                  int D, float scale, void* stream);
int afk_xattn_bwd(const void* Q, int64_t q_bs, int64_t q_hs, int64_t q_rs, const void* K, int64_t k_bs, int64_t k_hs,
                  int64_t k_rs, const void* V, int64_t v_bs, int64_t v_hs, int64_t v_rs, const void* dO,
                  int64_t do_bs, int64_t do_hs, int64_t do_rs, const void* Qt, const void* Kt, const void* dOt,
                  const float* LSE, const float* delta, void* dQ, int64_t dq_bs, int64_t dq_hs, int64_t dq_rs,
                  void* dK, int64_t dk_bs, int64_t dk_hs, int64_t dk_rs, void* dV, int64_t dv_bs, int64_t dv_hs,
                  int64_t dv_rs, const int* kv_len, const int* krange, int B, int Hq, int Hkv, int Sq, int Sk,
                  int Sqpad, int Skpad, int D, float scale, void* stream);

int afk_attn2_fwd(const void* Q, int64_t q_bs, int64_t q_hs, int64_t q_rs, const void* K, int64_t k_bs, int64_t k_hs,
                  int64_t k_rs, const void* V, int64_t v_bs, int64_t v_hs, int64_t v_rs, void* O, int64_t o_bs,
                  int64_t o_hs, int64_t o_rs, float* LSE, const int* kv_len, const int* kv_lo, int B, int Hq, int Hkv, int S, int Spad,
                  int D, float scale, int causal, void* stream);
int afk_attn_set_sched(int sched);
int afk_attn_set_xcd_map(int on);
int afk_attn_set_persist_paired(int on);
int afk_attn_set_dkdv_parts(int parts);
int afk_attn2_fwd_persistent(const void* Q, int64_t q_bs, int64_t q_hs, int64_t q_rs, const void* K, int64_t k_bs, int64_t k_hs,
                             int64_t k_rs, const void* V, int64_t v_bs, int64_t v_hs, int64_t v_rs, void* O, int64_t o_bs,
                             int64_t o_hs, int64_t o_rs, float* LSE, const int* kv_len, const int* kv_lo, int B, int Hq, int Hkv, int S, int Spad,
                             int D, float scale, int causal, int* queue, void* stream);
int afk_attn2_delta(const void* O, int64_t o_bs, int64_t o_hs, int64_t o_rs, const void* dO, int64_t do_bs, int64_t do_hs,
                    int64_t do_rs, float* delta, int B, int H, int S, int Spad, int D, void* stream);
int afk_attn2_bwd(const void* Q, int64_t q_bs, int64_t q_hs, int64_t q_rs, const void* K, int64_t k_bs, int64_t k_hs,
                  int64_t k_rs, const void* V, int64_t v_bs, int64_t v_hs, int64_t v_rs, const void* dO, int64_t do_bs,
                  int64_t do_hs, int64_t do_rs, const float* LSE, const float* delta, void* dQ, int64_t dq_bs,
                  int64_t dq_hs, int64_t dq_rs, void* dK, int64_t dk_bs, int64_t dk_hs, int64_t dk_rs, void* dV,
                  int64_t dv_bs, int64_t dv_hs, int64_t dv_rs, const int* kv_len, const int* kv_lo, int B, int Hq, int Hkv, int S,
                  int Spad, int D, float scale, int causal, void* gqa_scratch, void* stream);
int afk_attn2_bwd_fused(const void* Q, int64_t q_bs, int64_t q_hs, int64_t q_rs, const void* K, int64_t k_bs, int64_t k_hs,
                        int64_t k_rs, const void* V, int64_t v_bs, int64_t v_hs, int64_t v_rs, const void* O, int64_t o_bs, int64_t o_hs,
                        int64_t o_rs, const void* dO, int64_t do_bs, int64_t do_hs, int64_t do_rs, const float* LSE, float* delta_ws,
                        void* dQ, int64_t dq_bs, int64_t dq_hs, int64_t dq_rs, void* dK, int64_t dk_bs, int64_t dk_hs, int64_t dk_rs,
                        void* dV, int64_t dv_bs, int64_t dv_hs, int64_t dv_rs, const int* kv_len, const int* kv_lo, int B, int Hq,
                        int Hkv, int S, int Spad, int D, float scale, int causal, void* gqa_scratch, void* stream);
int afk_attn2_bwd_fused_rope(const void* Q, int64_t q_bs, int64_t q_hs, int64_t q_rs, const void* K, int64_t k_bs, int64_t k_hs,
                             int64_t k_rs, const void* V, int64_t v_bs, int64_t v_hs, int64_t v_rs, const void* O, int64_t o_bs, int64_t o_hs,
                             int64_t o_rs, const void* dO, int64_t do_bs, int64_t do_hs, int64_t do_rs, const float* LSE, float* delta_ws,
                             void* dQ, int64_t dq_bs, int64_t dq_hs, int64_t dq_rs, void* dK, int64_t dk_bs, int64_t dk_hs, int64_t dk_rs,
                             void* dV, int64_t dv_bs, int64_t dv_hs, int64_t dv_rs, const int* kv_len, const int* kv_lo, int B, int Hq,
                             int Hkv, int S, int Spad, int D, float scale, int causal, void* gqa_scratch, const void* cos_t, const void* sin_t,
                             const int* pos, const void* cos_lanes, const void* sin_lanes, void* stream);
int afk_rope_lanes_table(const void* table, void* out, int rows, int D, int form, void* stream);

int afk_rotary_time(const void* x, const float* cos_t, const float* sin_t, void* y, int64_t rows, int E, int R, int backward,
                    void* stream);

int afk_kv_cache_append(const void* qkv, int64_t ld, int k_col0, void* kcache, int64_t kc_bs, void* vtcache, int64_t vt_bs,
                        int spad, const int* start_dev, int start_host, int B, int n, int Hkv, int D, void* stream);

int afk_attn_decode_workspace_floats(int B, int Hq, int D, int nsplit);
int afk_attn_decode(const void* Q, int64_t q_bs, int64_t q_hs, const void* Kc, int64_t k_bs, int64_t k_rs, int64_t k_hs,
                    const void* Vt, int64_t vt_bs, int spad, void* O, int64_t o_bs, int64_t o_hs, const int* krange, int B,
                    int Hq, int Hkv, int D, float scale, int nsplit, float* workspace, void* stream);
int afk_attn_decode_fused(const void* Q, int64_t q_bs, int64_t q_hs, const void* Kc, int64_t k_bs, int64_t k_rs, int64_t k_hs,
                          const void* Vt, int64_t vt_bs, int spad, void* O, int64_t o_bs, int64_t o_hs, const int* krange, int B,
                          int Hq, int Hkv, int D, float scale, int nsplit, float* workspace, void* stream);
int afk_attn_decode_set_group(int mode);

int afk_gemv_partials(const void* A, int64_t lda, const void* B, int64_t ldb, int M, int N, int K, int splits, float* workspace,
                      void* stream);
int afk_decode_qkv_finish(const float* ws, int splits, int M, const void* bias, const void* cos_t, const void* sin_t, const int* pos,
                          void* q_out, void* kcache, int64_t kc_bs, void* vtcache, int64_t vt_bs, int spad, const int* start_dev,
                          int Hq, int Hkv, int D, void* stream);
int afk_decode_residual_rmsnorm(const float* ws, int splits, int M, int N, const void* residual, const void* w, float eps, void* x_out,
                                void* h_out, void* stream);
int afk_decode_swiglu(const float* ws, int splits, int M, int I, void* a_out, void* stream);

int afk_decode_chain_qkv(const void* x, const void* norm_w, float eps, const void* W, int64_t ldw, int K, const void* bias, const void* cos_t,
                         const void* sin_t, const int* pos, void* q_out, void* kcache, void* vtcache, int spad, const int* start_dev, int Hq,
                         int Hkv, int D, void* stream);
int afk_decode_chain_linear_residual(const void* x, const void* W, int64_t ldw, int N, int K, const void* residual, void* out, void* stream);
int afk_decode_chain_gate_up(const void* x, const void* norm_w, float eps, const void* W, int64_t ldw, int I, int K, void* act_out, void* stream);
int afk_decode_chain_lm_head(const void* x, const void* norm_w, float eps, const void* W, int64_t ldw, int N, int K, float* logits, float* part_val, int* part_idx,
                             void* stream);
int afk_decode_select_greedy(const float* part_val, const int* part_idx, int nparts, int64_t* next_token, int64_t* tokens_out, int tok_off, int* state,
                             const void* emb, int64_t ld_emb, int H, void* x_out, void* stream);
#define AFK_SAMPLE_MAX_V 8388608
int afk_decode_sample(const float* logits, int64_t ld_logits, int B, int V, float temperature, int top_k, float top_p, const float* u, int64_t seed,
                      const int* step_base, int step_off, int64_t* next_token, float* probs_out, int64_t ld_probs, int* kept_out, int64_t* tokens_out, int tok_off,
                      int* state, const void* emb, int64_t ld_emb, int H, void* x_out, void* stream);
int afk_decode_chain_qkv_batched(const void* h, int64_t ldh, int M, const void* W, int64_t ldw, int K, const void* bias, const void* cos_t, const void* sin_t,
                                 const int* pos, void* q_out, int64_t ldq, void* kcache, int64_t k_bs, void* vtcache, int64_t vt_bs, int spad, const int* start_dev,
                                 int Hq, int Hkv, int D, void* stream);
int afk_decode_chain_linear_residual_batched(const void* x, int64_t ldx, int M, const void* W, int64_t ldw, int N, int K, const void* residual, int64_t ld_res,
                                             void* out, int64_t ld_out, void* stream);
int afk_decode_chain_qkv_norm_batched(const void* x, int64_t ldx, int M, const void* norm_w, float eps, const void* W, int64_t ldw, int K, const void* bias,
                                      const void* cos_t, const void* sin_t, const int* pos, void* q_out, int64_t ldq, void* kcache, int64_t k_bs, void* vtcache,
                                      int64_t vt_bs, int spad, const int* start_dev, int Hq, int Hkv, int D, const float* ss_part, int ss_nparts, void* stream);
int afk_decode_chain_gate_up_norm_batched(const void* x, int64_t ldx, int M, const void* norm_w, float eps, const void* W, int64_t ldw, int I, int K, void* act_out,
                                          int64_t ld_act, const float* ss_part, int ss_nparts, void* stream);
int afk_decode_chain_lm_head_norm_batched(const void* x, int64_t ldx, int M, const void* norm_w, float eps, const void* W, int64_t ldw, int N, int K, float* logits,
                                          int64_t ld_logits, const float* ss_part, int ss_nparts, void* stream);
int afk_decode_chain_linear_residual_ss_batched(const void* x, int64_t ldx, int M, const void* W, int64_t ldw, int N, int K, const void* residual, int64_t ld_res,
                                                void* out, int64_t ld_out, float* ss_part, void* stream);
int afk_decode_chain_linear_residual_norm_batched(const void* x, int64_t ldx, int M, const void* W, int64_t ldw, int N, int K, const void* residual, int64_t ld_res,
                                                  void* out, int64_t ld_out, const void* norm_w, float eps, void* h_out, int64_t ld_h, int* counter, void* stream);
int afk_decode_chain_gate_up_batched(const void* h, int64_t ldh, int M, const void* W, int64_t ldw, int I, int K, void* act_out, int64_t ld_act, void* stream);
int afk_decode_chain_lm_head_batched(const void* h, int64_t ldh, int M, const void* W, int64_t ldw, int N, int K, float* logits, int64_t ld_logits, void* stream);

int afk_ce_fwd_bwd(void* logits, int64_t ld, int64_t rows, int V, const int64_t* shift_labels, float* row_loss,
                   const float* denom, float upstream, int write_grad, void* stream);
int afk_count_valid(const int64_t* labels, int64_t n, float* out, void* stream);
int afk_loss_reduce(const float* row_loss, int64_t n, const float* denom, float* loss, int accumulate, void* stream);

int afk_logmel(const float* wav, int W, int64_t nsamp, const float* cosb, const float* sinb, int nbins_pad,
               const float* melT, int nmel, float* raw_ws, int* wmax_ws, void* out, int out_is_bf16, void* stream);

int afk_adamw_step(float* master, float* m, float* v, const void* grad, void* param, int64_t n, float lr, float beta1,
                   float beta2, float eps, float weight_decay, int step, float grad_scale, int max_blocks, const int* gate,
                   const float* hyper, void* stream);
int afk_adamw_step_t(float* master, float* m, float* v, const void* grad, void* param, void* shadow, int N, int K, int64_t ld_shadow, float lr,
                     float beta1, float beta2, float eps, float weight_decay, int step, float grad_scale, int max_blocks, const int* gate,
                     const float* hyper, void* stream);
int afk_adamw16_step(void* m, void* v, const void* grad, void* param, int64_t n, double lr, double beta1, double beta2, double eps,
                     double weight_decay, int step, float grad_scale, int max_blocks, const int* gate, const float* hyper, void* stream);
int afk_adamw16_step_t(void* m, void* v, const void* grad, void* param, void* shadow, int N, int K, int64_t ld_shadow, double lr,
                       double beta1, double beta2, double eps, double weight_decay, int step, float grad_scale, int max_blocks,
                       const int* gate, const float* hyper, void* stream);
int afk_set_f32(float* dst, int n, float a, float b, float c, float d, void* stream);
int afk_sumsq_workspace_floats(void);
int afk_sumsq_bf16(const void* x, int64_t n, float* acc, const int* gate, float* workspace, void* stream);
int afk_clip_coef(const float* sumsq, int n, float scale, float max_norm, float* coef, float* norm_out, void* stream);

#define AFK_COMM_UID_BYTES 128
#define AFK_COMM_BF16 0
#define AFK_COMM_F32 1
#define AFK_COMM_I32 2
int afk_comm_unique_id(char* host_out128);
int afk_comm_init(int rank, int world, const char* host_uid128, void** host_comm_out);
int afk_comm_destroy(void* comm);
int afk_allreduce_bucket(void* comm, void* buf, int64_t n, int dtype, int op_max, void* stream);
int afk_reduce_scatter_allgather_bucket(void* comm, void* buf, int64_t n, int dtype, void* stream);
int64_t afk_comm_share(int64_t n, int world, int dtype);
int afk_reduce_scatter_bucket(void* comm, void* buf, int64_t n, int dtype, void* stream);
int afk_allgather_bucket(void* comm, void* buf, int64_t n, int dtype, void* stream);
int afk_comm_broadcast(void* comm, void* buf, int64_t n, int dtype, int root, void* stream);
int afk_cu_hog(int nblocks, int lds_bytes, const int* stop_flag, int64_t max_ticks, int64_t* report, void* stream);

int afk_mfma_ceiling(int mode, int nblocks, int iters, const void* operands, float* sink, double* host_flops, void* stream);

int afk_stream_priority_range(int* host_least, int* host_greatest);
int afk_stream_create(int priority, void** host_stream_out);
int afk_stream_create_cu_mask(int first_cu, int n_cus, void** host_stream_out);
int afk_stream_destroy(void* stream);

int afk_x32_linear(const float* A, int64_t lda, const void* W, int64_t ldw, float* C, int64_t ldc, int M, int N, int K, const void* bias,
                   const float* residual, int64_t ldr, int res_mod, float alpha, int gelu, void* stream);
int afk_x32_norm(const float* x, const void* w, const void* b, float* y, int64_t rows, int D, float eps, int rms, void* stream);
int afk_x32_attention(const float* Q, int64_t ldq, const float* K, int64_t ldk, const float* V, int64_t ldv, float* O, int64_t ldo, int B, int S, int Hq,
                      int Hkv, int D, float scale, int causal, const int* kv_lo, const int* kv_len, void* stream);
int afk_x32_rope(float* x, int64_t ld, const float* cos_tab, const float* sin_tab, int64_t rows, int S, int nheads, int D, void* stream);
int afk_x32_silu_mul(const float* gate_up, float* out, int64_t rows, int I, void* stream);
int afk_x32_conv3_gelu(const float* x, int x_cmajor, const void* w, const void* bias, const void* pos, float* y, int W, int C, int T, int E, int stride,
                       void* stream);
int afk_x32_avgpool2(const float* x, float* y, int64_t W, int T, int E, void* stream);
int afk_x32_embed_scatter(const int64_t* ids, const int* src, const float* audio, const void* embed, float* out, int64_t rows, int H, void* stream);

#ifdef __cplusplus
}
#endif
#endif
```

Before: 600.2 audio-s/s.

## Add 16x16x32 MFMA variant of 256-tile GEMM and make it default for NT

Templates the 256x256 GEMM kernels on MFMA shape, adding a v_mfma_f32_16x16x32_bf16 path with its own fragment addressing, accumulator layout and permlane16 epilogue. A dispatch rule now selects 16x16x32 for the NT form by default, keeping 32x32x16 for NN/TN, with env and API overrides. The intent is better MFMA issue efficiency or LDS read pattern on MI355X for the forward GEMMs, at the cost of more accumulator registers and extra reshuffling in the epilogue. The ceiling microbenchmark gains matching 16x16 modes.

```diff
diff --git a/audio-flamingo_amd/csrc/ceiling.hip b/audio-flamingo_amd/csrc/ceiling.hip
--- a/audio-flamingo_amd/csrc/ceiling.hip
+++ b/audio-flamingo_amd/csrc/ceiling.hip
@@ -5,7 +5,7 @@
 
 constexpr int SEG = 16;
 
-template <int MODE>
+template <int MODE, int MF>
 __global__ __launch_bounds__(512, 1) void mfma_ceiling_kernel(const bf16* __restrict__ src, float* __restrict__ sink, int iters) {
     extern __shared__ __attribute__((aligned(16))) char smem[];
     const int tid = threadIdx.x, lane = tid & 63, wave = tid >> 6;
@@ -23,12 +23,19 @@
         __syncthreads();
     }
     f32x16 acc[2][2];
+    f32x4 acc16[4][4];
 #pragma unroll
     for (int i = 0; i < 2; ++i)
 #pragma unroll
         for (int j = 0; j < 2; ++j)
 #pragma unroll
             for (int e = 0; e < 16; ++e) acc[i][j][e] = 0.f;
+#pragma unroll
+    for (int i = 0; i < 4; ++i)
+#pragma unroll
+        for (int j = 0; j < 4; ++j)
+#pragma unroll
+            for (int e = 0; e < 4; ++e) acc16[i][j][e] = 0.f;
     uint32_t lds = afk_lds_addr(smem) + lane * 16;
     for (int it = 0; it < iters; ++it) {
         if (MODE == 1) {
@@ -41,14 +48,30 @@
             });
             afk_lds_wait0(a[0][0], a[0][1], a[0][2], a[0][3], a[1][0], a[1][1], a[1][2], a[1][3], b[0][0], b[1][1], b[0][2], b[1][3]);
         }
+        if constexpr (MF == 32) {
 #pragma unroll
-        for (int k = 0; k < 4; ++k)
+            for (int k = 0; k < 4; ++k)
 #pragma unroll
-            for (int i = 0; i < 2; ++i)
+                for (int i = 0; i < 2; ++i)
 #pragma unroll
-                for (int j = 0; j < 2; ++j) acc[i][j] = __builtin_amdgcn_mfma_f32_32x32x16_bf16(a[i][k], b[j][k], acc[i][j], 0, 0, 0);
+                    for (int j = 0; j < 2; ++j) acc[i][j] = __builtin_amdgcn_mfma_f32_32x32x16_bf16(a[i][k], b[j][k], acc[i][j], 0, 0, 0);
+        } else {
+#pragma unroll
+            for (int k = 0; k < 2; ++k)
+#pragma unroll
+                for (int i = 0; i < 4; ++i)
+#pragma unroll
+                    for (int j = 0; j < 4; ++j)
+                        acc16[i][j] = __builtin_amdgcn_mfma_f32_16x16x32_bf16(a[i >> 1][2 * (i & 1) + k], b[j >> 1][2 * (j & 1) + k], acc16[i][j], 0, 0, 0);
+        }
     }
     float s = 0.f;
+#pragma unroll
+    for (int i = 0; i < 4; ++i)
+#pragma unroll
+        for (int j = 0; j < 4; ++j)
+#pragma unroll
+            for (int e = 0; e < 4; ++e) s += acc16[i][j][e];
 #pragma unroll
     for (int i = 0; i < 2; ++i)
 #pragma unroll
@@ -101,11 +124,11 @@
 }
 
 extern "C" int afk_mfma_ceiling(int mode, int nblocks, int iters, const void* operands, float* sink, double* host_flops, void* stream) {
-    AFK_REQUIRE(mode >= 0 && mode <= 3, "afk_mfma_ceiling: mode %d (0 = register-resident operands, 1 = + LDS fragment reads, 2 / 3 = issue pacing of one wave per SIMD, "
-                "independent / dependent accumulators: sink[0] = cycles per MFMA)", mode);
+    AFK_REQUIRE(mode >= 0 && mode <= 5, "afk_mfma_ceiling: mode %d (0 = register-resident operands, 1 = + LDS fragment reads, 2 / 3 = issue pacing of one wave per SIMD, "
+                "independent / dependent accumulators: sink[0] = cycles per MFMA, 4 / 5 = modes 0 / 1 on v_mfma_f32_16x16x32_bf16)", mode);
     AFK_REQUIRE(nblocks > 0 && iters > 0 && operands && sink, "afk_mfma_ceiling: bad arguments");
     hipStream_t s = (hipStream_t)stream;
-    if (mode >= 2) {
+    if (mode == 2 || mode == 3) {
         if (mode == 2) mfma_pacing_kernel<false><<<nblocks, 256, 0, s>>>((const bf16*)operands, sink, iters);
         else mfma_pacing_kernel<true><<<nblocks, 256, 0, s>>>((const bf16*)operands, sink, iters);
         AFK_LAUNCH_CHECK("afk_mfma_ceiling");
@@ -113,14 +136,18 @@
         return AFK_OK;
     }
     if (mode == 0) {
-        mfma_ceiling_kernel<0><<<nblocks, 512, 0, s>>>((const bf16*)operands, sink, iters);
+        mfma_ceiling_kernel<0, 32><<<nblocks, 512, 0, s>>>((const bf16*)operands, sink, iters);
+    } else if (mode == 4) {
+        mfma_ceiling_kernel<0, 16><<<nblocks, 512, 0, s>>>((const bf16*)operands, sink, iters);
     } else {
         static bool attr = false;
         if (!attr) {
-            hipFuncSetAttribute((const void*)mfma_ceiling_kernel<1>, hipFuncAttributeMaxDynamicSharedMemorySize, 65536 + 16384);
+            hipFuncSetAttribute((const void*)mfma_ceiling_kernel<1, 32>, hipFuncAttributeMaxDynamicSharedMemorySize, 65536 + 16384);
+            hipFuncSetAttribute((const void*)mfma_ceiling_kernel<1, 16>, hipFuncAttributeMaxDynamicSharedMemorySize, 65536 + 16384);
             attr = true;
         }
-        mfma_ceiling_kernel<1><<<nblocks, 512, 65536 + 16384, s>>>((const bf16*)operands, sink, iters);
+        if (mode == 1) mfma_ceiling_kernel<1, 32><<<nblocks, 512, 65536 + 16384, s>>>((const bf16*)operands, sink, iters);
+        else mfma_ceiling_kernel<1, 16><<<nblocks, 512, 65536 + 16384, s>>>((const bf16*)operands, sink, iters);
     }
     AFK_LAUNCH_CHECK("afk_mfma_ceiling");
     if (host_flops) *host_flops = (double)nblocks * 8.0 * iters * SEG * 2.0 * 32 * 32 * 16;
diff --git a/audio-flamingo_amd/csrc/gemm.hip b/audio-flamingo_amd/csrc/gemm.hip
--- a/audio-flamingo_amd/csrc/gemm.hip
+++ b/audio-flamingo_amd/csrc/gemm.hip
@@ -99,7 +99,7 @@
 #pragma unroll
     for (int i = 0; i < 2; ++i)
 #pragma unroll
-        for (int j = 0; j < 2; ++j) gemm_store_block32_body<-1>(p, m0 + wm * 64 + i * 32 + l31, n0 + wn * 64 + j * 32, hi, acc[i][j]);
+        for (int j = 0; j < 2; ++j) gemm_store_block32_body<-1, 32>(p, m0 + wm * 64 + i * 32, n0 + wn * 64 + j * 32, lane, acc[i][j]);
 }
 
 #define AFK_GEMV_MAX_M 1
@@ -196,6 +196,20 @@
 [[maybe_unused]] int g_256_impl = 2;
 int g_gm = 0;
 int g_wide = 1;
+int g_mfma = 0;
+
+constexpr int mfma_shapes(int form) { return form == 0 ? AFK_MFMA_SHAPES_NT : form == 1 ? AFK_MFMA_SHAPES_NN : AFK_MFMA_SHAPES_TN; }
+constexpr int AFK_MFMA_RULE_NT = 16, AFK_MFMA_RULE_NN = 32, AFK_MFMA_RULE_TN = 32;
+int gemm_mfma_of(int form) {
+    static const int env = [] {
+        const char* e = getenv("AFK_GEMM_MFMA");
+        return (e && e[0] >= '0' && e[0] <= '2' && !e[1]) ? e[0] - '0' : 0;
+    }();
+    const int sel = g_mfma ? g_mfma : env;
+    if (sel == 1) return 32;
+    if (sel == 2) return 16;
+    return form == 0 ? AFK_MFMA_RULE_NT : form == 1 ? AFK_MFMA_RULE_NN : AFK_MFMA_RULE_TN;
+}
 
 hipEvent_t prof_next_event() {
     if (g_prof.used == g_prof.pool.size()) {
@@ -221,6 +235,16 @@
     g_variant = base;
     return AFK_OK;
 }
+
+extern "C" int afk_gemm_set_mfma(int v) {
+    AFK_REQUIRE(v >= 0 && v <= 2, "afk_gemm_set_mfma: %d (0 = dispatch rule, 1 = 32x32x16, 2 = 16x16x32)", v);
+    constexpr int any = AFK_MFMA_SHAPES_NT | AFK_MFMA_SHAPES_NN | AFK_MFMA_SHAPES_TN;
+    AFK_REQUIRE(v == 0 || (any >> (v - 1)) & 1, "afk_gemm_set_mfma: no 256x256 kernel of this libafk.so carries the %s shape; build with make PROBES=1",
+                v == 1 ? "32x32x16" : "16x16x32");
+    g_mfma = v;
+    return AFK_OK;
+}
+extern "C" int afk_gemm_mfma_shapes(int form) { return form >= 0 && form <= 2 ? mfma_shapes(form) : 0; }
 
 extern "C" int afk_prof_enable(int on) {
     std::lock_guard<std::mutex> lk(g_prof.mu);
@@ -371,7 +395,7 @@
         if (g > 2048) g = 2048;
         hipLaunchKernelGGL(gemm_splitk_reduce_kernel, dim3(g), dim3(256), 0, st, p);
     } else if (trans_b) {
-        if (int e = afk_launch_gemm256t(p, trans_a, st)) return e;
+        if (int e = afk_launch_gemm256t(p, trans_a, gemm_mfma_of(trans_a ? 2 : 1), st)) return e;
         if (splits > 1) {
             int g = (int)afk_cdiv((int64_t)M * (N / 4), 256);
             if (g > 2048) g = 2048;
@@ -379,9 +403,9 @@
         }
     } else if (use256) {
 #ifdef AFK_PROBES
-        if (int e = persist_q ? afk_launch_gemm256q(p, st) : persist ? afk_launch_gemm256p(p, st) : f8 ? afk_launch_gemm256f8(p, impl256 - 10, st) : w4 ? afk_launch_gemm256w4(p, impl256 - 3, st) : afk_launch_gemm256(p, st)) return e;
+        if (int e = persist_q ? afk_launch_gemm256q(p, st) : persist ? afk_launch_gemm256p(p, st) : f8 ? afk_launch_gemm256f8(p, impl256 - 10, st) : w4 ? afk_launch_gemm256w4(p, impl256 - 3, st) : afk_launch_gemm256(p, gemm_mfma_of(0), st)) return e;
 #else
-        if (int e = afk_launch_gemm256(p, st)) return e;
+        if (int e = afk_launch_gemm256(p, gemm_mfma_of(0), st)) return e;
 #endif
     } else {
         hipLaunchKernelGGL(gemm_nt_bf16_k128, dim3((unsigned)nwg, (unsigned)splits), dim3(256), NSTAGE * STAGE_BYTES, st, p);
diff --git a/audio-flamingo_amd/csrc/gemm256.hip b/audio-flamingo_amd/csrc/gemm256.hip
--- a/audio-flamingo_amd/csrc/gemm256.hip
+++ b/audio-flamingo_amd/csrc/gemm256.hip
@@ -17,7 +17,7 @@
         __builtin_amdgcn_sched_barrier(0);    \
     } while (0)
 
-template <int EPI>
+template <int EPI, int MF>
 __global__ __launch_bounds__(512, 1) void gemm_nt_bf16_k256(GemmArgs p) {
     extern __shared__ __attribute__((aligned(16))) char smem[];
     const int tid = threadIdx.x;
@@ -78,20 +78,14 @@
             __builtin_amdgcn_global_load_lds((gbl_void*)(ysrc[j] + koff), (lds_void*)(base + ydst[j]), 16, 0, 0);
     };
 
-    const int swz_l = (lane >> 1) & 7;
     int koffb[4];
 #pragma unroll
-    for (int s = 0; s < 4; ++s) koffb[s] = ((2 * s + hi) ^ swz_l) << 4;
-    const int a_row0 = (wm * 128 + l31) * ROWB;
-    const int b_row0 = OP_BYTES + (wn * 64 + l31) * ROWB;
-
-    f32x16 acc[4][2];
-#pragma unroll
-    for (int i = 0; i < 4; ++i)
-#pragma unroll
-        for (int j = 0; j < 2; ++j)
-#pragma unroll
-            for (int e = 0; e < 16; ++e) acc[i][j][e] = 0.f;
+    for (int x = 0; x < 4; ++x) koffb[x] = gemm_frag_rowoff<MF>(x) * ROWB + gemm_frag_koff<MF>(x, lane);
+    const int a_row0 = (wm * 128 + gemm_frag_row<MF>(lane)) * ROWB;
+    const int b_row0 = OP_BYTES + (wn * 64 + gemm_frag_row<MF>(lane)) * ROWB;
+
+    GemmAcc<MF> acc;
+    acc.zero();
 
     const int T = p.K / BK;
     issue_x(0);
@@ -106,11 +100,35 @@
     if (wm == 1) AFK_BARRIER();
 
     bf16x8 bf[2][4], af[2][4];
-#define AFK_MFMA4(ACC0, s)                                                                                         \
-    do {                                                                                                           \
-        _Pragma("unroll") for (int i_ = 0; i_ < 2; ++i_) _Pragma("unroll") for (int j_ = 0; j_ < 2; ++j_)          \
-            acc[ACC0 + i_][j_] = __builtin_amdgcn_mfma_f32_32x32x16_bf16(bf[j_][s], af[i_][s], acc[ACC0 + i_][j_], 0, 0, 0); \
-    } while (0)
+    auto mfma_group = [&](auto acc0_, auto g_) {
+        constexpr int ACC0 = decltype(acc0_)::value, g = decltype(g_)::value;
+        if constexpr (MF == 32) {
+#pragma unroll
+            for (int i = 0; i < 2; ++i)
+#pragma unroll
+                for (int j = 0; j < 2; ++j) acc.mma(ACC0 + i, j, bf[j][g], af[i][g]);
+        } else {
+            constexpr int s = g >> 1, i = g & 1;
+#pragma unroll
+            for (int ih = 0; ih < 2; ++ih)
+#pragma unroll
+                for (int jt = 0; jt < 4; ++jt) acc.mma(2 * (ACC0 + i) + ih, jt, bf[jt >> 1][2 * (jt & 1) + s], af[i][2 * ih + s]);
+        }
+    };
+    auto mfma_slot = [&](auto acc0_, auto q_) {
+        constexpr int ACC0 = decltype(acc0_)::value, q = decltype(q_)::value;
+        if constexpr (MF == 32) {
+            constexpr int s = q >> 1, i = q & 1;
+            acc.mma(ACC0 + i, 0, bf[0][s], af[i][s]);
+            acc.mma(ACC0 + i, 1, bf[1][s], af[i][s]);
+        } else {
+            constexpr int s = q >> 2, i = (q >> 1) & 1, ih = q & 1;
+#pragma unroll
+            for (int jt = 0; jt < 4; ++jt) acc.mma(2 * (ACC0 + i) + ih, jt, bf[jt >> 1][2 * (jt & 1) + s], af[i][2 * ih + s]);
+        }
+    };
+    using afk_c2 = std::integral_constant<int, 2>;
+#define AFK_MFMA4(ACC0, g) mfma_group(std::integral_constant<int, ACC0>{}, std::integral_constant<int, g>{})
     for (int t = 0; t < T; ++t) {
         const char* buf = smem + (t & 1) * BUF_BYTES;
         const int t1 = min(t + 1, T - 1), t2 = min(t + 2, T - 1);
@@ -151,20 +169,15 @@
         AFK_VMCNT(2);
         AFK_BARRIER();
         __builtin_amdgcn_s_setprio(1);
-#pragma unroll
-        for (int s = 0; s < 4; ++s) {
-#pragma unroll
-            for (int i = 0; i < 2; ++i) {
-                acc[2 + i][0] = __builtin_amdgcn_mfma_f32_32x32x16_bf16(bf[0][s], af[i][s], acc[2 + i][0], 0, 0, 0);
-                acc[2 + i][1] = __builtin_amdgcn_mfma_f32_32x32x16_bf16(bf[1][s], af[i][s], acc[2 + i][1], 0, 0, 0);
-                const int piece = 2 * s + i;
-                if (piece < 6) {
-                    __builtin_amdgcn_sched_barrier(0);
-                    __builtin_amdgcn_global_load_lds((gbl_void*)(xsrc[piece] + ox), (lds_void*)(bx + xdst[piece]), 16, 0, 0);
-                    __builtin_amdgcn_sched_barrier(0);
-                }
+        afk_static_for<8>([&](auto q_) {
+            constexpr int piece = decltype(q_)::value;
+            mfma_slot(afk_c2{}, q_);
+            if constexpr (piece < 6) {
+                __builtin_amdgcn_sched_barrier(0);
+                __builtin_amdgcn_global_load_lds((gbl_void*)(xsrc[piece] + ox), (lds_void*)(bx + xdst[piece]), 16, 0, 0);
+                __builtin_amdgcn_sched_barrier(0);
             }
-        }
+        });
         __builtin_amdgcn_s_setprio(0);
         AFK_VMCNT(8);
         AFK_BARRIER();
@@ -186,12 +199,14 @@
             for (int j = 0; j < 2; ++j)
 #pragma unroll
                 for (int t = 0; t < 2; ++t) {
+                    const f32x16 blk = acc.block(i, j);
                     b8 o;
 #pragma unroll
                     for (int e = 0; e < 4; ++e) {
-                        const auto r = __builtin_amdgcn_permlane32_swap(__float_as_uint(acc[i][j][8 * t + e]), __float_as_uint(acc[i][j][8 * t + 4 + e]), false, false);
-                        o[e] = (bf16)(__uint_as_float(r[0]) * p.alpha);
-                        o[4 + e] = (bf16)(__uint_as_float(r[1]) * p.alpha);
+                        float v0, v1;
+                        gemm_lane_swap<MF>(blk[8 * t + e], blk[8 * t + 4 + e], v0, v1);
+                        o[e] = (bf16)(v0 * p.alpha);
+                        o[4 + e] = (bf16)(v1 * p.alpha);
                     }
                     pc[(i * 2 + j) * 2 + t] = o;
                 }
@@ -239,11 +254,14 @@
                     const int n = n0 + wn * 64 + j * 32 + 16 * t + 8 * hi;
                     b8 bv;
                     if constexpr ((EPI & AFK_GEMM_BIAS) != 0) bv = *(const b8*)(p.bias + n);
+                    const f32x16 blk = acc.block(i, j);
                     b8 o;
 #pragma unroll
                     for (int e = 0; e < 4; ++e) {
-                        const auto r = __builtin_amdgcn_permlane32_swap(__float_as_uint(acc[i][j][8 * t + e]), __float_as_uint(acc[i][j][8 * t + 4 + e]), false, false);
-                        float v0 = __uint_as_float(r[0]) * p.alpha, v1 = __uint_as_float(r[1]) * p.alpha;
+                        float v0, v1;
+                        gemm_lane_swap<MF>(blk[8 * t + e], blk[8 * t + 4 + e], v0, v1);
+                        v0 *= p.alpha;
+                        v1 *= p.alpha;
                         if constexpr ((EPI & AFK_GEMM_BIAS) != 0) {
                             v0 += (float)bv[e];
                             v1 += (float)bv[4 + e];
@@ -291,7 +309,7 @@
 #pragma unroll
     for (int i = 0; i < 4; ++i)
 #pragma unroll
-        for (int j = 0; j < 2; ++j) gemm_store_block32<EPI>(p, m0 + wm * 128 + i * 32 + l31, n0 + wn * 64 + j * 32, hi, acc[i][j]);
+        for (int j = 0; j < 2; ++j) gemm_store_block32<EPI, MF>(p, m0 + wm * 128 + i * 32, n0 + wn * 64 + j * 32, lane, acc.block(i, j));
 }
 
 }
@@ -299,11 +317,12 @@
 #define AFK_EPI_LIST(X) X(0) X(AFK_GEMM_BIAS) X(AFK_GEMM_RESIDUAL) X(AFK_GEMM_BIAS | AFK_GEMM_RESIDUAL) X(AFK_GEMM_BIAS | AFK_GEMM_GELU) \
     X(AFK_GEMM_BIAS | AFK_GEMM_GELU | AFK_GEMM_RESIDUAL) X(AFK_GEMM_ACCUM) X(AFK_GEMM_SWIGLU_FWD) X(AFK_GEMM_SWIGLU_BWD) X(AFK_GEMM_ROPE) X(AFK_GEMM_ROPE | AFK_GEMM_BIAS) X(-1)
 
-int afk_launch_gemm256(const GemmArgs& p, hipStream_t st) {
+template <int MF>
+static int launch_gemm256(const GemmArgs& p, hipStream_t st) {
     static bool attr_set = false;
     if (!attr_set) {
-#define AFK_SET(F)                                                                                                                       \
-    if (hipFuncSetAttribute((const void*)gemm_nt_bf16_k256<(F)>, hipFuncAttributeMaxDynamicSharedMemorySize, LDS_BYTES) != hipSuccess) \
+#define AFK_SET(F)                                                                                                                           \
+    if (hipFuncSetAttribute((const void*)gemm_nt_bf16_k256<(F), MF>, hipFuncAttributeMaxDynamicSharedMemorySize, LDS_BYTES) != hipSuccess) \
         return afk_set_error(AFK_ERR_LAUNCH, "gemm256: cannot reserve %d bytes of LDS", LDS_BYTES);
         AFK_EPI_LIST(AFK_SET)
 #undef AFK_SET
@@ -312,16 +331,24 @@
     const int64_t nwg = (int64_t)p.ntm * p.ntn;
     const int f = (p.wide && p.splits <= 1) ? p.flags : -1;
     switch (f) {
-#define AFK_CASE(F)                                                                                          \
-    case (F):                                                                                                \
-        if ((F) == -1) afk_count(AFK_CNT_GEMM_GENERIC);                                                      \
-        hipLaunchKernelGGL(gemm_nt_bf16_k256<(F)>, dim3((unsigned)nwg), dim3(512), LDS_BYTES, st, p);        \
+#define AFK_CASE(F)                                                                                              \
+    case (F):                                                                                                    \
+        if ((F) == -1) afk_count(AFK_CNT_GEMM_GENERIC);                                                          \
+        hipLaunchKernelGGL((gemm_nt_bf16_k256<(F), MF>), dim3((unsigned)nwg), dim3(512), LDS_BYTES, st, p);      \
         break;
         AFK_EPI_LIST(AFK_CASE)
 #undef AFK_CASE
         default:
             afk_count(AFK_CNT_GEMM_GENERIC);
-            hipLaunchKernelGGL(gemm_nt_bf16_k256<-1>, dim3((unsigned)nwg), dim3(512), LDS_BYTES, st, p);
+            hipLaunchKernelGGL((gemm_nt_bf16_k256<-1, MF>), dim3((unsigned)nwg), dim3(512), LDS_BYTES, st, p);
     }
     return AFK_OK;
 }
+
+int afk_launch_gemm256(const GemmArgs& p, int mf, hipStream_t st) {
+    if constexpr ((AFK_MFMA_SHAPES_NT & 2) != 0)
+        if (mf == 16) return launch_gemm256<16>(p, st);
+    if constexpr ((AFK_MFMA_SHAPES_NT & 1) != 0)
+        if (mf == 32) return launch_gemm256<32>(p, st);
+    return afk_set_error(AFK_ERR_UNSUPPORTED, "gemm256: the %s MFMA shape of the NT kernel is built under make PROBES=1 only", mf == 16 ? "16x16x32" : "32x32x16");
+}
diff --git a/audio-flamingo_amd/csrc/gemm256t.hip b/audio-flamingo_amd/csrc/gemm256t.hip
--- a/audio-flamingo_amd/csrc/gemm256t.hip
+++ b/audio-flamingo_amd/csrc/gemm256t.hip
@@ -24,19 +24,19 @@
         __builtin_amdgcn_global_load_lds((gbl_void*)(SRCPTR), (lds_void*)(DSTPTR), 16, 0, 0);             \
         __builtin_amdgcn_sched_barrier(0);                                                                \
     } while (0)
-#define MFMA(a, b, c) __builtin_amdgcn_mfma_f32_32x32x16_bf16(a, b, c, 0, 0, 0)
 
 __device__ __forceinline__ int tswz(int r) { return ((r & 3) << 2) | ((r >> 2) & 3); }
 
-__device__ __forceinline__ int tr_off(int tile32, int pc, int lane) {
-    const int g = lane >> 4, i = lane & 15, hi = g >> 1;
-    const int chunk = 4 * tile32 + 2 * (g & 1) + ((i & 3) >> 1);
-    const int r = 8 * hi + (i >> 2) + 4 * pc;
+template <int MF>
+__device__ __forceinline__ int tr_off(int tile, int pc, int lane) {
+    const int g = lane >> 4, i = lane & 15;
+    const int chunk = MF == 16 ? 2 * tile + ((i & 3) >> 1) : 4 * tile + 2 * (g & 1) + ((i & 3) >> 1);
+    const int r = (MF == 16 ? 8 * g : 8 * (g >> 1)) + (i >> 2) + 4 * pc;
     return r * TROW + ((chunk ^ tswz(r)) << 4) + 8 * (i & 1);
 }
-template <int S>
+template <int MF, int S>
 __device__ __forceinline__ bf16x8 tr_frag(uint32_t buf, int off0, int off1) {
-    return afk_lds_tr_frag<S * 16 * TROW>(buf + off0, buf + off1);
+    return afk_lds_tr_frag<S * (48 - MF) * TROW>(buf + off0, buf + off1);
 }
 
 struct TSrc {
@@ -54,7 +54,7 @@
     return s;
 }
 
-template <bool AT, int EPI>
+template <bool AT, int EPI, int MF>
 __global__ __launch_bounds__(512, 1) void gemm_xt_bf16_k256(GemmArgs p) {
     extern __shared__ __attribute__((aligned(16))) char smem[];
     const int tid = threadIdx.x;
@@ -116,13 +116,8 @@
     const bf16* tbase[NX + NY];
 #pragma unroll
     for (int j = 0; j < NX + NY; ++j) tbase[j] = (AT || j < 4) ? tr_src[j].base + (int64_t)tr_src[j].krow * tr_ld[j] : nullptr;
-    f32x16 acc[4][2];
-#pragma unroll
-    for (int i = 0; i < 4; ++i)
-#pragma unroll
-        for (int j = 0; j < 2; ++j)
-#pragma unroll
-            for (int e = 0; e < 16; ++e) acc[i][j][e] = 0.f;
+    GemmAcc<MF> acc;
+    acc.zero();
 
     const bool ragged = (KL % BK) != 0;
   auto pipeline = [&](auto rag_) {
@@ -141,20 +136,30 @@
     };
     auto issue = [&](int j, int t_src, int parity) { AFK_DMA_PTR(src_of(j, t_src), smem + parity * BUF_BYTES + dst[j]); };
 
-    int tob[2][2], toa[4][2];
+    constexpr int NH = MF == 16 ? 2 : 1;
+    int tob[2][NH][2], toa[4][NH][2];
 #pragma unroll
     for (int j = 0; j < 2; ++j)
 #pragma unroll
-        for (int pc = 0; pc < 2; ++pc) tob[j][pc] = OP_BYTES + tr_off(wn * 2 + j, pc, lane);
+        for (int h = 0; h < NH; ++h)
+#pragma unroll
+            for (int pc = 0; pc < 2; ++pc) tob[j][h][pc] = OP_BYTES + tr_off<MF>((wn * 2 + j) * NH + h, pc, lane);
 #pragma unroll
     for (int i = 0; i < 4; ++i)
 #pragma unroll
-        for (int pc = 0; pc < 2; ++pc) toa[i][pc] = AT ? tr_off(wm * 4 + i, pc, lane) : 0;
-    const int swz_l = (lane >> 1) & 7;
+        for (int h = 0; h < NH; ++h)
+#pragma unroll
+            for (int pc = 0; pc < 2; ++pc) toa[i][h][pc] = AT ? tr_off<MF>((wm * 4 + i) * NH + h, pc, lane) : 0;
+    auto tr_read = [&](uint32_t lbuf, const int (&to)[NH][2], auto x_, auto ks0_) {
+        constexpr int x = decltype(x_)::value, ks0 = decltype(ks0_)::value;
+        if constexpr (MF == 32) return tr_frag<MF, ks0 + x>(lbuf, to[0][0], to[0][1]);
+        else if constexpr (AT) return tr_frag<MF, ks0>(lbuf, to[x][0], to[x][1]);
+        else return tr_frag<MF, (x & 1)>(lbuf, to[x >> 1][0], to[x >> 1][1]);
+    };
     int koffb[4];
 #pragma unroll
-    for (int s = 0; s < 4; ++s) koffb[s] = ((2 * s + hi) ^ swz_l) << 4;
-    const int a_row0 = (wm * 128 + l31) * 128;
+    for (int x = 0; x < 4; ++x) koffb[x] = gemm_frag_rowoff<MF>(x) * 128 + gemm_frag_koff<MF>(x, lane);
+    const int a_row0 = (wm * 128 + gemm_frag_row<MF>(lane)) * 128;
 
 #pragma unroll
     for (int j = 0; j < NX; ++j) issue(j, 0, 0);
@@ -176,10 +181,10 @@
         const uint32_t lbuf = lds0 + (t & 1) * BUF_BYTES;
         const int t1 = min(t + 1, T - 1), t2 = min(t + 2, T - 1);
         const int e1 = (t + 1) & 1, e2 = t & 1;
-        if (!AT) {
+        if constexpr (!AT) {
 #pragma unroll
             for (int j = 0; j < 2; ++j)
-                afk_static_for<4>([&](auto s_) { constexpr int s = decltype(s_)::value; bf[j][s] = tr_frag<s>(lbuf, tob[j][0], tob[j][1]); });
+                afk_static_for<4>([&](auto x_) { bf[j][decltype(x_)::value] = tr_read(lbuf, tob[j], x_, std::integral_constant<int, 0>{}); });
 #pragma unroll
             for (int i = 0; i < 2; ++i)
 #pragma unroll
@@ -188,14 +193,22 @@
             AFK_VMCNT(6);
             AFK_BARRIER();
             __builtin_amdgcn_s_setprio(1);
-#pragma unroll
-            for (int s = 0; s < 4; ++s) {
-#pragma unroll
-                for (int i = 0; i < 2; ++i)
-#pragma unroll
-                    for (int j = 0; j < 2; ++j) acc[i][j] = MFMA(bf[j][s], af[i][s], acc[i][j]);
-                if (s < 2) issue(NX + s, t1, e1);
-            }
+            afk_static_for<4>([&](auto g_) {
+                constexpr int g = decltype(g_)::value;
+                if constexpr (MF == 32) {
+#pragma unroll
+                    for (int i = 0; i < 2; ++i)
+#pragma unroll
+                        for (int j = 0; j < 2; ++j) acc.mma(i, j, bf[j][g], af[i][g]);
+                } else {
+                    constexpr int s = g >> 1, i = g & 1;
+#pragma unroll
+                    for (int ih = 0; ih < 2; ++ih)
+#pragma unroll
+                        for (int jt = 0; jt < 4; ++jt) acc.mma(2 * i + ih, jt, bf[jt >> 1][2 * (jt & 1) + s], af[i][2 * ih + s]);
+                }
+                if constexpr (g < 2) issue(NX + g, t1, e1);
+            });
             __builtin_amdgcn_s_setprio(0);
             AFK_VMCNT(8);
             AFK_BARRIER();
@@ -207,16 +220,19 @@
             AFK_VMCNT(2);
             AFK_BARRIER();
             __builtin_amdgcn_s_setprio(1);
-#pragma unroll
-            for (int s = 0; s < 4; ++s) {
-#pragma unroll
-                for (int i = 0; i < 2; ++i) {
-                    acc[2 + i][0] = MFMA(bf[0][s], af[i][s], acc[2 + i][0]);
-                    acc[2 + i][1] = MFMA(bf[1][s], af[i][s], acc[2 + i][1]);
-                    const int piece = 2 * s + i;
-                    if (piece < 6) issue(piece, t2, e2);
+            afk_static_for<8>([&](auto q_) {
+                constexpr int piece = decltype(q_)::value;
+                if constexpr (MF == 32) {
+                    constexpr int s = piece >> 1, i = piece & 1;
+                    acc.mma(2 + i, 0, bf[0][s], af[i][s]);
+                    acc.mma(2 + i, 1, bf[1][s], af[i][s]);
+                } else {
+                    constexpr int s = piece >> 2, i = (piece >> 1) & 1, ih = piece & 1;
+#pragma unroll
+                    for (int jt = 0; jt < 4; ++jt) acc.mma(2 * (2 + i) + ih, jt, bf[jt >> 1][2 * (jt & 1) + s], af[i][2 * ih + s]);
                 }
-            }
+                if constexpr (piece < 6) issue(piece, t2, e2);
+            });
             __builtin_amdgcn_s_setprio(0);
             AFK_VMCNT(8);
             AFK_BARRIER();
@@ -224,18 +240,19 @@
             const int kvalid = KL - t * BK;
 #pragma unroll
             for (int ph = 0; ph < 2; ++ph) {
-                afk_static_for<2>([&](auto s_) {
-                    constexpr int s = decltype(s_)::value;
+                afk_static_for<2>([&](auto x_) {
+                    constexpr int x = decltype(x_)::value;
+                    constexpr int KS = MF == 16 ? 1 : 2;
                     if (ph == 0) {
 #pragma unroll
-                        for (int j = 0; j < 2; ++j) bf[j][s] = tr_frag<s>(lbuf, tob[j][0], tob[j][1]);
-#pragma unroll
-                        for (int i = 0; i < 4; ++i) af[i][s] = tr_frag<s>(lbuf, toa[i][0], toa[i][1]);
+                        for (int j = 0; j < 2; ++j) bf[j][x] = tr_read(lbuf, tob[j], x_, std::integral_constant<int, 0>{});
+#pragma unroll
+                        for (int i = 0; i < 4; ++i) af[i][x] = tr_read(lbuf, toa[i], x_, std::integral_constant<int, 0>{});
                     } else {
 #pragma unroll
-                        for (int j = 0; j < 2; ++j) bf[j][s] = tr_frag<2 + s>(lbuf, tob[j][0], tob[j][1]);
-#pragma unroll
-                        for (int i = 0; i < 4; ++i) af[i][s] = tr_frag<2 + s>(lbuf, toa[i][0], toa[i][1]);
+                        for (int j = 0; j < 2; ++j) bf[j][x] = tr_read(lbuf, tob[j], x_, std::integral_constant<int, KS>{});
+#pragma unroll
+                        for (int i = 0; i < 4; ++i) af[i][x] = tr_read(lbuf, toa[i], x_, std::integral_constant<int, KS>{});
                     }
                 });
                 AFK_LGKMCNT0();
@@ -244,7 +261,7 @@
                     for (int s = 0; s < 2; ++s)
 #pragma unroll
                         for (int e = 0; e < 8; ++e) {
-                            const bool dead = 16 * (2 * ph + s) + 8 * hi + e >= kvalid;
+                            const bool dead = (MF == 16 ? 32 * ph + 8 * (lane >> 4) : 16 * (2 * ph + s) + 8 * hi) + e >= kvalid;
 #pragma unroll
                             for (int i = 0; i < 4; ++i)
                                 if (dead) af[i][s][e] = (bf16)0.f;
@@ -253,19 +270,22 @@
                 AFK_VMCNT(4);
                 AFK_BARRIER();
                 __builtin_amdgcn_s_setprio(1);
-#pragma unroll
-                for (int s = 0; s < 2; ++s) {
-#pragma unroll
-                    for (int i = 0; i < 4; ++i) {
-                        acc[i][0] = MFMA(bf[0][s], af[i][s], acc[i][0]);
-                        acc[i][1] = MFMA(bf[1][s], af[i][s], acc[i][1]);
-                        const int piece = 4 * s + i;
-                        if ((piece & 1) == 0) {
-                            if (ph == 0) issue(NX + (piece >> 1), t1, e1);
-                            else issue(piece >> 1, t2, e2);
-                        }
+                afk_static_for<8>([&](auto q_) {
+                    constexpr int piece = decltype(q_)::value;
+                    if constexpr (MF == 32) {
+                        constexpr int s = piece >> 2, i = piece & 3;
+                        acc.mma(i, 0, bf[0][s], af[i][s]);
+                        acc.mma(i, 1, bf[1][s], af[i][s]);
+                    } else {
+                        constexpr int i = piece >> 1, ih = piece & 1;
+#pragma unroll
+                        for (int jt = 0; jt < 4; ++jt) acc.mma(2 * i + ih, jt, bf[jt >> 1][jt & 1], af[i][ih]);
                     }
-                }
+                    if constexpr ((piece & 1) == 0) {
+                        if (ph == 0) issue(NX + (piece >> 1), t1, e1);
+                        else issue(piece >> 1, t2, e2);
+                    }
+                });
                 __builtin_amdgcn_s_setprio(0);
                 AFK_VMCNT(8);
                 AFK_BARRIER();
@@ -281,19 +301,19 @@
 #pragma unroll
     for (int i = 0; i < 4; ++i)
 #pragma unroll
-        for (int j = 0; j < 2; ++j) gemm_store_block32<EPI>(p, m0 + wm * 128 + i * 32 + l31, n0 + wn * 64 + j * 32, hi, acc[i][j]);
+        for (int j = 0; j < 2; ++j) gemm_store_block32<EPI, MF>(p, m0 + wm * 128 + i * 32, n0 + wn * 64 + j * 32, lane, acc.block(i, j));
 }
 
 }
 
 #define AFK_EPI_LIST(X) X(0) X(AFK_GEMM_ACCUM) X(-2) X(-1)
 
-int afk_launch_gemm256t(const GemmArgs& p, int trans_a, hipStream_t st) {
+template <bool AT, int MF>
+static int launch_gemm256t(const GemmArgs& p, hipStream_t st) {
     static bool attr_set = false;
     if (!attr_set) {
-#define AFK_SET(F)                                                                                                                                \
-    if (hipFuncSetAttribute((const void*)gemm_xt_bf16_k256<false, (F)>, hipFuncAttributeMaxDynamicSharedMemorySize, LDS_BYTES) != hipSuccess || \
-        hipFuncSetAttribute((const void*)gemm_xt_bf16_k256<true, (F)>, hipFuncAttributeMaxDynamicSharedMemorySize, LDS_BYTES) != hipSuccess)    \
+#define AFK_SET(F)                                                                                                                              \
+    if (hipFuncSetAttribute((const void*)gemm_xt_bf16_k256<AT, (F), MF>, hipFuncAttributeMaxDynamicSharedMemorySize, LDS_BYTES) != hipSuccess) \
         return afk_set_error(AFK_ERR_LAUNCH, "gemm256t: cannot reserve %d bytes of LDS", LDS_BYTES);
         AFK_EPI_LIST(AFK_SET)
 #undef AFK_SET
@@ -304,18 +324,32 @@
     const int f = p.splits > 1 ? -2 : (p.wide ? p.flags : -1);
     const dim3 grid((unsigned)nwg, ns);
     switch (f) {
-#define AFK_CASE(F)                                                                                                   \
-    case (F):                                                                                                         \
-        if ((F) == -1) afk_count(AFK_CNT_GEMM_GENERIC);                                                               \
-        if (trans_a) hipLaunchKernelGGL((gemm_xt_bf16_k256<true, (F)>), grid, dim3(512), LDS_BYTES, st, p);          \
-        else hipLaunchKernelGGL((gemm_xt_bf16_k256<false, (F)>), grid, dim3(512), LDS_BYTES, st, p);                 \
+#define AFK_CASE(F)                                                                                        \
+    case (F):                                                                                              \
+        if ((F) == -1) afk_count(AFK_CNT_GEMM_GENERIC);                                                    \
+        hipLaunchKernelGGL((gemm_xt_bf16_k256<AT, (F), MF>), grid, dim3(512), LDS_BYTES, st, p);           \
         break;
         AFK_EPI_LIST(AFK_CASE)
 #undef AFK_CASE
         default:
             afk_count(AFK_CNT_GEMM_GENERIC);
-            if (trans_a) hipLaunchKernelGGL((gemm_xt_bf16_k256<true, -1>), grid, dim3(512), LDS_BYTES, st, p);
-            else hipLaunchKernelGGL((gemm_xt_bf16_k256<false, -1>), grid, dim3(512), LDS_BYTES, st, p);
+            hipLaunchKernelGGL((gemm_xt_bf16_k256<AT, -1, MF>), grid, dim3(512), LDS_BYTES, st, p);
     }
     return AFK_OK;
 }
+
+int afk_launch_gemm256t(const GemmArgs& p, int trans_a, int mf, hipStream_t st) {
+    if (trans_a) {
+        if constexpr ((AFK_MFMA_SHAPES_TN & 2) != 0)
+            if (mf == 16) return launch_gemm256t<true, 16>(p, st);
+        if constexpr ((AFK_MFMA_SHAPES_TN & 1) != 0)
+            if (mf == 32) return launch_gemm256t<true, 32>(p, st);
+    } else {
+        if constexpr ((AFK_MFMA_SHAPES_NN & 2) != 0)
+            if (mf == 16) return launch_gemm256t<false, 16>(p, st);
+        if constexpr ((AFK_MFMA_SHAPES_NN & 1) != 0)
+            if (mf == 32) return launch_gemm256t<false, 32>(p, st);
+    }
+    return afk_set_error(AFK_ERR_UNSUPPORTED, "gemm256t: the %s MFMA shape of the %s kernel is built under make PROBES=1 only", mf == 16 ? "16x16x32" : "32x32x16",
+                         trans_a ? "TN" : "NN");
+}
diff --git a/audio-flamingo_amd/csrc/gemm_common.h b/audio-flamingo_amd/csrc/gemm_common.h
--- a/audio-flamingo_amd/csrc/gemm_common.h
+++ b/audio-flamingo_amd/csrc/gemm_common.h
@@ -124,57 +124,145 @@
 }
 __device__ __forceinline__ void gemm_epilogue_store4(const GemmArgs& p, int m, int n, float v[4]) { gemm_epilogue_store<4, -1>(p, m, n, v); }
 
-template <int F>
-__device__ __forceinline__ void gemm_store_block32_body(const GemmArgs& p, int m, int nb, int hi, const f32x16& acc);
-static __device__ __noinline__ void gemm_store_block32_generic(const GemmArgs& p, int m, int nb, int hi, f32x16 acc) {
-    gemm_store_block32_body<-1>(p, m, nb, hi, acc);
-}
-template <int F = -1>
-__device__ __forceinline__ void gemm_store_block32(const GemmArgs& p, int m, int nb, int hi, const f32x16& acc) {
-    if constexpr (F == -1) gemm_store_block32_generic(p, m, nb, hi, acc);
-    else gemm_store_block32_body<F>(p, m, nb, hi, acc);
-}
-template <int F>
-__device__ __forceinline__ void gemm_store_block32_body(const GemmArgs& p, int m, int nb, int hi, const f32x16& acc) {
-    if (m >= p.M) return;
+template <int MF>
+__device__ __forceinline__ int gemm_frag_row(int lane) { return MF == 16 ? (lane & 15) : (lane & 31); }
+template <int MF>
+__device__ __forceinline__ int gemm_frag_koff(int x, int lane) {
+    const int chunk = MF == 16 ? 4 * (x & 1) + (lane >> 4) : 2 * x + (lane >> 5);
+    return (chunk ^ ((lane >> 1) & 7)) << 4;
+}
+template <int MF>
+__device__ __forceinline__ constexpr int gemm_frag_rowoff(int x) { return MF == 16 ? (x >> 1) * 16 : 0; }
+
+template <int MF>
+struct GemmAcc;
+template <>
+struct GemmAcc<32> {
+    f32x16 v[4][2];
+    __device__ __forceinline__ void zero() {
+#pragma unroll
+        for (int i = 0; i < 4; ++i)
+#pragma unroll
+            for (int j = 0; j < 2; ++j)
+#pragma unroll
+                for (int e = 0; e < 16; ++e) v[i][j][e] = 0.f;
+    }
+    __device__ __forceinline__ void mma(int i, int j, const bf16x8& b, const bf16x8& a) { v[i][j] = __builtin_amdgcn_mfma_f32_32x32x16_bf16(b, a, v[i][j], 0, 0, 0); }
+    __device__ __forceinline__ f32x16 block(int i, int j) const { return v[i][j]; }
+};
+template <>
+struct GemmAcc<16> {
+    f32x4 v[8][4];
+    __device__ __forceinline__ void zero() {
+#pragma unroll
+        for (int i = 0; i < 8; ++i)
+#pragma unroll
+            for (int j = 0; j < 4; ++j)
+#pragma unroll
+                for (int e = 0; e < 4; ++e) v[i][j][e] = 0.f;
+    }
+    __device__ __forceinline__ void mma(int it, int jt, const bf16x8& b, const bf16x8& a) { v[it][jt] = __builtin_amdgcn_mfma_f32_16x16x32_bf16(b, a, v[it][jt], 0, 0, 0); }
+    __device__ __forceinline__ f32x16 block(int i, int j) const {
+        f32x16 b;
+#pragma unroll
+        for (int t = 0; t < 2; ++t)
+#pragma unroll
+            for (int h = 0; h < 2; ++h)
+#pragma unroll
+                for (int e = 0; e < 4; ++e) b[8 * t + 4 * h + e] = v[2 * i + h][2 * j + t][e];
+        return b;
+    }
+};
+
+template <int MF>
+__device__ __forceinline__ void gemm_lane_swap(float x, float y, float& lo, float& hi) {
+    if constexpr (MF == 16) {
+        const auto r = __builtin_amdgcn_permlane16_swap(__float_as_uint(x), __float_as_uint(y), false, false);
+        lo = __uint_as_float(r[0]);
+        hi = __uint_as_float(r[1]);
+    } else {
+        const auto r = __builtin_amdgcn_permlane32_swap(__float_as_uint(x), __float_as_uint(y), false, false);
+        lo = __uint_as_float(r[0]);
+        hi = __uint_as_float(r[1]);
+    }
+}
+template <int MF>
+__device__ __forceinline__ void gemm_quad_pos(int lane, int t, int h, int& row, int& col) {
+    if (MF == 16) {
+        row = 16 * h + (lane & 15);
+        col = 16 * t + 4 * (lane >> 4);
+    } else {
+        row = lane & 31;
+        col = 8 * (2 * t + h) + 4 * (lane >> 5);
+    }
+}
+
+template <int F, int MF>
+__device__ __forceinline__ void gemm_store_block32_body(const GemmArgs& p, int mb, int nb, int lane, const f32x16& b);
+template <int MF>
+static __device__ __noinline__ void gemm_store_block32_generic(const GemmArgs& p, int mb, int nb, int lane, f32x16 b) {
+    gemm_store_block32_body<-1, MF>(p, mb, nb, lane, b);
+}
+template <int F = -1, int MF = 32>
+__device__ __forceinline__ void gemm_store_block32(const GemmArgs& p, int mb, int nb, int lane, const f32x16& b) {
+    if constexpr (F == -1) gemm_store_block32_generic<MF>(p, mb, nb, lane, b);
+    else gemm_store_block32_body<F, MF>(p, mb, nb, lane, b);
+}
+template <int F, int MF>
+__device__ __forceinline__ void gemm_store_block32_body(const GemmArgs& p, int mb, int nb, int lane, const f32x16& b) {
     if (F == -2 || (F == -1 && p.splits > 1)) {
 #pragma unroll
-        for (int q = 0; q < 4; ++q) {
-            const int n = nb + 8 * q + 4 * hi;
-            if (n >= p.N) continue;
-            const f32x4 o = {acc[4 * q], acc[4 * q + 1], acc[4 * q + 2], acc[4 * q + 3]};
-            *(f32x4*)(p.ws + ((int64_t)blockIdx.y * p.M + m) * p.N + n) = o;
-        }
+        for (int t = 0; t < 2; ++t)
+#pragma unroll
+            for (int h = 0; h < 2; ++h) {
+                int row, col;
+                gemm_quad_pos<MF>(lane, t, h, row, col);
+                const int m = mb + row, n = nb + col;
+                if (m >= p.M || n >= p.N) continue;
+                const f32x4 o = {b[8 * t + 4 * h], b[8 * t + 4 * h + 1], b[8 * t + 4 * h + 2], b[8 * t + 4 * h + 3]};
+                *(f32x4*)(p.ws + ((int64_t)blockIdx.y * p.M + m) * p.N + n) = o;
+            }
         return;
     }
     if constexpr (F == -2) return;
     if (F >= 0 || p.wide) {
+        const int m = mb + (lane & 31);
 #pragma unroll
         for (int t = 0; t < 2; ++t) {
             float v[8];
 #pragma unroll
-            for (int e = 0; e < 4; ++e) {
-                const auto r = __builtin_amdgcn_permlane32_swap(__float_as_uint(acc[8 * t + e]), __float_as_uint(acc[8 * t + 4 + e]), false, false);
-                v[e] = __uint_as_float(r[0]);
-                v[4 + e] = __uint_as_float(r[1]);
-            }
-            const int n = nb + 16 * t + 8 * hi;
-            if (n < p.N) gemm_epilogue_store<8, F>(p, m, n, v);
+            for (int e = 0; e < 4; ++e) gemm_lane_swap<MF>(b[8 * t + e], b[8 * t + 4 + e], v[e], v[4 + e]);
+            const int n = nb + 16 * t + 8 * (lane >> 5);
+            if (m < p.M && n < p.N) gemm_epilogue_store<8, F>(p, m, n, v);
         }
         return;
     }
 #pragma unroll
-    for (int q = 0; q < 4; ++q) {
-        const int n = nb + 8 * q + 4 * hi;
-        if (n >= p.N) continue;
-        float v[4] = {acc[4 * q], acc[4 * q + 1], acc[4 * q + 2], acc[4 * q + 3]};
-        gemm_epilogue_store<4, F>(p, m, n, v);
-    }
-}
-
-int afk_launch_gemm256(const GemmArgs& p, hipStream_t st);
+    for (int t = 0; t < 2; ++t)
+#pragma unroll
+        for (int h = 0; h < 2; ++h) {
+            int row, col;
+            gemm_quad_pos<MF>(lane, t, h, row, col);
+            const int m = mb + row, n = nb + col;
+            if (m >= p.M || n >= p.N) continue;
+            float v[4] = {b[8 * t + 4 * h], b[8 * t + 4 * h + 1], b[8 * t + 4 * h + 2], b[8 * t + 4 * h + 3]};
+            gemm_epilogue_store<4, F>(p, m, n, v);
+        }
+}
+
+#ifdef AFK_PROBES
+#define AFK_MFMA_SHAPES_NT 3
+#define AFK_MFMA_SHAPES_NN 3
+#define AFK_MFMA_SHAPES_TN 3
+#else
+#define AFK_MFMA_SHAPES_NT 2
+#define AFK_MFMA_SHAPES_NN 1
+#define AFK_MFMA_SHAPES_TN 1
+#endif
+
+int afk_launch_gemm256(const GemmArgs& p, int mf, hipStream_t st);
 int afk_launch_gemm256p(const GemmArgs& p, hipStream_t st);
 int afk_launch_gemm256q(const GemmArgs& p, hipStream_t st);
 int afk_launch_gemm256f8(const GemmArgs& p, int mode, hipStream_t st);
 int afk_launch_gemm256w4(const GemmArgs& p, int mode, hipStream_t st);
-int afk_launch_gemm256t(const GemmArgs& p, int trans_a, hipStream_t st);
+int afk_launch_gemm256t(const GemmArgs& p, int trans_a, int mf, hipStream_t st);
diff --git a/audio-flamingo_amd/ops.py b/audio-flamingo_amd/ops.py
--- a/audio-flamingo_amd/ops.py
+++ b/audio-flamingo_amd/ops.py
@@ -760,6 +760,15 @@
     _lib.call("afk_gemm_set_variant", int(v))
 
 
+def gemm_set_mfma(v: int):
+    _lib.call("afk_gemm_set_mfma", int(v))
+
+
+def gemm_mfma_shapes(form: str) -> tuple:
+    mask = _lib.load().afk_gemm_mfma_shapes(("nt", "nn", "tn").index(form))
+    return tuple(v for v in (1, 2) if mask >> (v - 1) & 1)
+
+
 KERNEL_FAMILIES = ("gemm_nt128", "gemm_nt256", "gemm_nn256", "gemm_tn256", "gemm_splitk", "gemv", "attn2_fwd_d64", "attn2_fwd_d128",
                    "attn2_bwd_d64", "attn2_bwd_d128", "gqa_reduce", "xattn_fwd", "xattn_bwd", "attn1_fwd", "attn1_bwd", "gemm_generic_epilogue")
 
diff --git a/include/afk.h b/include/afk.h
--- a/include/afk.h
+++ b/include/afk.h
@@ -36,6 +36,8 @@
 int afk_prof_dump(const char* host_path);
 
 int afk_gemm_set_variant(int variant);
+int afk_gemm_set_mfma(int v);
+int afk_gemm_mfma_shapes(int form);
 #define AFK_GEMM_BIAS 1
 #define AFK_GEMM_GELU 2
 #define AFK_GEMM_RESIDUAL 4
```

Measured after the change: 607.6 audio-s/s (median of 6 runs). 1.01x the previous value.
